# JuliaQuantumControl/GRAPE.jl

Hardware: AMD Instinct MI355X
Metric: GRAPE gradient evals/sec (N=64, 1000 steps, 128 traj) (higher is better)
Workload: dtype f64

## Files before the change

### grape.jl_amd/api.py

```python
from __future__ import annotations

import ctypes as C
import os
import subprocess
import sys

import numpy as np

_HERE = os.path.dirname(os.path.abspath(__file__))
_CSRC = os.path.join(_HERE, "csrc")
_LIBNAME = "libgrape_hip.so"

J_T_SM, J_T_SS, J_T_RE = 0, 1, 2
GRAD_GRADGEN, GRAD_TAYLOR = 0, 1
PROP_EXP, PROP_SERIES = 0, 1
ABI_VERSION = 7

STATUS = {0: "GRAPE_OK", -1: "GRAPE_ERR_INVALID", -2: "GRAPE_ERR_HIP", -3: "GRAPE_ERR_CHI_NORM",
          -4: "GRAPE_ERR_SINGULAR", -5: "GRAPE_ERR_TAYLOR", -6: "GRAPE_ERR_NO_CONTROLS", -7: "GRAPE_ERR_AGAIN",
          -8: "GRAPE_ERR_HOST"}

EXPORTS = ["grape_create", "grape_destroy", "grape_eval", "grape_forward", "grape_backward",
           "grape_forward_device", "grape_backward_device", "grape_check", "grape_get_propagator",
           "grape_get_tau_grads", "grape_get_storage", "grape_get_timings", "grape_reset_timings", "grape_get_work", "grape_get_cert_table", "grape_get_seg_table",
           "grape_last_error", "grape_abi_version", "grape_set_fused_sweeps", "grape_get_sums", "grape_backward_xi",
           "grape_get_final_states", "grape_backward_chi",
           "grape_get_time_gradient", "grape_set_tlist", "grape_eval_batch", "grape_get_batch_info", "grape_create_open",
           "grape_hvp", "grape_get_hvp_info", "grape_open_time_gradient", "grape_open_hvp", "grape_get_open_hvp_info",
           "grape_open_eval_batch", "grape_get_open_batch_info", "grape_open_set_running_cost", "grape_open_backward_xi",
           "grape_hvp_forward", "grape_hvp_backward", "grape_hvp_backward_chi",
           "grape_open_hvp_forward", "grape_open_hvp_backward", "grape_open_hvp_backward_chi",
           "grape_expect", "grape_get_expect_info"]


class GrapeHipError(RuntimeError):
    def __init__(self, code, msg):
        super().__init__(f"{STATUS.get(code, code)}: {msg}")
        self.code = code


class _Problem(C.Structure):
    _fields_ = [("abi_version", C.c_int32), ("N", C.c_int32), ("L", C.c_int32), ("K", C.c_int32),
                ("K_total", C.c_int32), ("N_T", C.c_int32), ("functional", C.c_int32),
                ("gradient_method", C.c_int32), ("hc_per_traj", C.c_int32), ("device", C.c_int32),
                ("tlist", C.c_void_p), ("H0", C.c_void_p), ("Hc", C.c_void_p), ("shape", C.c_void_p),
                ("psi0", C.c_void_p), ("target", C.c_void_p), ("weights", C.c_void_p),
                ("chi_min_norm", C.c_double), ("taylor_max_order", C.c_int32),
                ("taylor_tolerance", C.c_double),
                ("Dpen", C.c_void_p), ("dpen_per_traj", C.c_int32), ("lambda_b", C.c_double),
                ("prop_method", C.c_int32), ("prop_tolerance", C.c_double),
                ("ndev", C.c_int32), ("devices", C.c_void_p), ("taylor_no_check", C.c_int32)]


class _Lindblad(C.Structure):
    _fields_ = [("J", C.c_int32), ("cops_per_traj", C.c_int32), ("cops", C.c_void_p)]


def library_path() -> str:
    return os.path.join(_CSRC, _LIBNAME)


def build_asm(verbose: bool = False, workdir: str | None = None) -> str:
    asm_dir = os.path.join(_CSRC, "asm")
    work = workdir or asm_dir
    kernels = (("gen_t16.py", "expm_t16_asm"), ("gen_t16q.py", "expm_t16q_asm"), ("gen_t16p.py", "expm_t16p_asm"), ("gen_t16p.py", "expm_t16p4_asm"), ("gen_t18g.py", "expm_t18g_asm"), ("gen_t18gp.py", "expm_t18gp_asm"), ("gen_d3.py", "deriv3_asm"), ("gen_d3s.py", "deriv3s_asm"), ("gen_d3s.py", "deriv3g_asm"),
               ("gen_lg.py", "lg_gemm_asm"), ("gen_d4.py", "deriv4_asm_128"), ("gen_d4.py", "deriv4_asm_256"))
    co_path, emb_s, emb_o = os.path.join(work, "grape_asm.co"), os.path.join(work, "asm_embed.S"), os.path.join(work, "asm_embed.o")
    llvm = "/opt/rocm/lib/llvm/bin"
    cmds, objs = [], []
    for gen_py, name in kernels:
        s_path, o_path = os.path.join(work, name + ".s"), os.path.join(work, name + ".o")
        gen = subprocess.run([sys.executable, os.path.join(asm_dir, gen_py), s_path], capture_output=True, text=True)
        if verbose or gen.returncode:
            print(gen.stdout, gen.stderr)
        if gen.returncode:
            raise RuntimeError(gen_py + " failed")
        cmds.append([os.path.join(llvm, "clang"), "-x", "assembler", "-target", "amdgcn-amd-amdhsa", "-mcpu=gfx950", "-c", s_path, "-o", o_path])
        objs.append(o_path)
    cmds.append([os.path.join(llvm, "ld.lld"), "-shared"] + objs + ["-o", co_path])
    with open(emb_s, "w") as f:
        f.write('\t.section .rodata\n\t.globl grape_asm_co_start\n\t.globl grape_asm_co_end\n\t.p2align 12\n'
                'grape_asm_co_start:\n\t.incbin "grape_asm.co"\ngrape_asm_co_end:\n\t.byte 0\n'
                '\t.section .note.GNU-stack,"",@progbits\n')
    cmds.append(["gcc", "-c", "-fPIC", "asm_embed.S", "-o", "asm_embed.o"])
    for c in cmds:
        res = subprocess.run(c, capture_output=True, text=True, cwd=work)
        if verbose or res.returncode:
            print(" ".join(c), res.stdout, res.stderr)
        if res.returncode:
            raise RuntimeError("assembling the gfx950 kernels failed")
    return emb_o


def _sources():
    srcs = [os.path.join(_CSRC, f) for f in ("grape_hip.hip", "grape_t18.hip", "grape_kernels.hip.h", "grape_large.hip.h",
                                             "grape_series.hip.h", "grape_cheby.hip.h", "grape_t18.hip.h", "grape_t18_coeffs.h",
                                             "grape_deriv3.hip.h", "grape_timegrad.hip.h", "grape_batch.hip.h", "grape_lindblad.hip.h", "grape_lindblad_tg.hip.h", "grape_hvp.hip.h", "grape_hvp_split.hip.h", "grape_lindblad_hvp.hip.h", "grape_lindblad_hvp_split.hip.h", "grape_lindblad_batch.hip.h", "grape_lindblad_rc.hip.h", "grape_devmem.h", "grape_cert.hip.h", "grape_expect.hip.h", "grape_econ_coeffs.h", os.path.join("asm", "gen_t16.py"), os.path.join("asm", "gen_t16q.py"), os.path.join("asm", "gen_t16p.py"), os.path.join("asm", "gen_t18g.py"), os.path.join("asm", "gen_t18gp.py"), os.path.join("asm", "gen_d3.py"), os.path.join("asm", "gen_d3s.py"), os.path.join("asm", "gen_lg.py"), os.path.join("asm", "gen_d4.py"), os.path.join("asm", "gcn.py"))]
    return srcs, os.path.join(_HERE, "..", "include", "grape_hip.h")


def _up_to_date(out: str) -> bool:
    srcs, hdr = _sources()
    return os.path.exists(out) and all(os.path.getmtime(out) >= os.path.getmtime(s) for s in srcs + [hdr])


def build_library(force: bool = False, verbose: bool = False, extra_flags=(), out: str | None = None) -> str:
    import fcntl
    import shutil
    import tempfile
    out = out or library_path()
    if not force and _up_to_date(out):
        return out
    srcs, _ = _sources()
    with open(os.path.join(_CSRC, ".build.lock"), "w") as lockf:
        fcntl.flock(lockf, fcntl.LOCK_EX)
        if not force and _up_to_date(out):
            return out
        work = tempfile.mkdtemp(prefix="_build_", dir=_CSRC)
        procs = []
        try:
            base = ["hipcc", "--offload-arch=gfx950", "-O3", "-std=c++17", "-fPIC", "-Wno-unused-value"] + list(extra_flags)
            objs = [os.path.join(work, "grape_hip.o"), os.path.join(work, "grape_t18.o")]
            cmds = [base + ["-cuid=grapehip0", "-c", srcs[0], "-o", objs[0]],
                    base + ["-cuid=grapehip1", "-mllvm", "-amdgpu-mfma-vgpr-form", "-c", srcs[1], "-o", objs[1]]]
            procs = [subprocess.Popen(c, stdout=subprocess.PIPE, stderr=subprocess.STDOUT, text=True) for c in cmds]
            objs.append(build_asm(verbose, workdir=work))
            outs = [p.communicate()[0] for p in procs]
            if verbose or any(p.returncode for p in procs):
                print("\n".join(outs))
            if any(p.returncode for p in procs):
                raise RuntimeError("hipcc failed building " + out)
            tmp_so = os.path.join(work, _LIBNAME)
            res = subprocess.run(["hipcc", "--offload-arch=gfx950", "-shared", "-fPIC"] + objs + ["-o", tmp_so], capture_output=True, text=True)
            if verbose or res.returncode:
                print(res.stdout, res.stderr)
            if res.returncode:
                raise RuntimeError("hipcc failed linking " + out)
            asm_dir = os.path.join(_CSRC, "asm")
            for f in os.listdir(work):
                if f.endswith(".s") or f.endswith(".co"):
                    os.replace(os.path.join(work, f), os.path.join(asm_dir, f))
            os.replace(tmp_so, out)
        finally:
            for p in procs:
                if p.poll() is None:
                    p.kill()
                    p.communicate()
            shutil.rmtree(work, ignore_errors=True)
    return out


_lib = None


def load_library():
    global _lib
    if _lib is not None:
        return _lib
    path = library_path()
    if not os.path.exists(path):
        raise GrapeHipError(-2, f"{path} not built; run __graft_entry__.build() (no CPU fallback exists)")
    try:
        import torch
    except ImportError:
        pass
    lib = C.CDLL(path)
    vp, dp, ip = C.c_void_p, C.POINTER(C.c_double), C.c_int
    lib.grape_create.argtypes = [C.POINTER(vp), C.POINTER(_Problem)]
    lib.grape_create_open.argtypes = [C.POINTER(vp), C.POINTER(_Problem), C.POINTER(_Lindblad)]
    lib.grape_destroy.argtypes = [vp]
    lib.grape_destroy.restype = None
    lib.grape_eval.argtypes = [vp, vp, dp, vp, vp, vp]
    lib.grape_forward.argtypes = [vp, vp, vp]
    lib.grape_backward.argtypes = [vp, vp, vp]
    lib.grape_forward_device.argtypes = [vp, vp, vp, vp]
    lib.grape_backward_device.argtypes = [vp, vp, vp, vp]
    lib.grape_check.argtypes = [vp, vp]
    lib.grape_get_propagator.argtypes = [vp, ip, ip, vp]
    lib.grape_get_tau_grads.argtypes = [vp, vp]
    lib.grape_get_storage.argtypes = [vp, ip, vp]
# ... 251 lines not shown

    def hvp_forward(self, V, final_states=False):
        v, nv = self._hvp_dirs(V)
        dtau = np.empty((nv, self.K), dtype=np.complex128)
        dsums = np.empty(nv, dtype=np.complex128)
        dpsi = np.empty((nv, self.K, self.N), dtype=np.complex128) if final_states else None
        self._chk(self._lib.grape_hvp_forward(self._h, nv, v.ctypes.data, dtau.ctypes.data, dsums.ctypes.data,
                                              dpsi.ctypes.data if final_states else None))
        if v.ndim == 1:
            dtau, dsums, dpsi = dtau[0], dsums[0], (dpsi[0] if final_states else None)
        return (dtau, dsums, dpsi) if final_states else (dtau, dsums)

    def hvp_backward(self, f_total, df_total):
        one = np.ndim(df_total) == 0
        df = np.ascontiguousarray(df_total, dtype=np.complex128)
        if np.ndim(df_total) > 1 or df.size == 0:
            raise ValueError(f"df_total must be a complex scalar or [nv] with nv >= 1, got {np.shape(df_total)}")
        nv = df.size
        out = np.empty((nv, self.L * self.N_T))
        f = np.array([complex(f_total).real, complex(f_total).imag], dtype=np.float64)
        self._chk(self._lib.grape_hvp_backward(self._h, nv, f.ctypes.data, df.ctypes.data, out.ctypes.data))
        return out[0] if one else out

    def hvp_backward_chi(self, chi, dchi):
        chi = np.ascontiguousarray(chi, dtype=np.complex128)
        d = np.ascontiguousarray(dchi, dtype=np.complex128)
        if chi.shape != (self.K, self.N):
            raise ValueError(f"chi must be [K, N] = [{self.K}, {self.N}], got {chi.shape}")
        if d.ndim not in (2, 3) or d.shape[-2:] != (self.K, self.N) or d.size == 0:
            raise ValueError(f"dchi must be [K, N] = [{self.K}, {self.N}] or [nv, {self.K}, {self.N}] with nv >= 1, got {d.shape}")
        nv = 1 if d.ndim == 2 else d.shape[0]
        out = np.empty((nv, self.L * self.N_T))
        self._chk(self._lib.grape_hvp_backward_chi(self._h, nv, chi.ctypes.data, d.ctypes.data, out.ctypes.data))
        return out[0] if d.ndim == 2 else out

    def set_tlist(self, tlist):
        t = np.ascontiguousarray(tlist, dtype=np.float64)
        if t.shape != (self.N_T + 1,):
            raise ValueError(f"tlist must have N_T + 1 = {self.N_T + 1} points, got {t.shape}")
        self._chk(self._lib.grape_set_tlist(self._h, t.ctypes.data))
        self._tlist = t

    def forward_device(self, d_pulsevals_ptr, d_out_ptr, stream=0):
        self._chk(self._lib.grape_forward_device(self._h, d_pulsevals_ptr, d_out_ptr, stream))

    def backward_device(self, d_f_ptr, d_G_ptr, stream=0):
        self._chk(self._lib.grape_backward_device(self._h, d_f_ptr, d_G_ptr, stream))

    def set_fused_sweeps(self, on=True):
        return bool(self._lib.grape_set_fused_sweeps(self._h, int(bool(on))))

    def check(self, stream=0):
        self._chk(self._lib.grape_check(self._h, stream))

    def propagator(self, k, n):
        out = np.empty((self.N, self.N), dtype=np.complex128)
        self._chk(self._lib.grape_get_propagator(self._h, k, n, out.ctypes.data))
        return out.T.copy()

    def tau_grads(self):
        out = np.empty((self.K, self.L, self.N_T), dtype=np.complex128)
        self._chk(self._lib.grape_get_tau_grads(self._h, out.ctypes.data))
        return out

    def storage(self, which=0):
        out = np.empty((self.K, self.N_T + 1, self.N), dtype=np.complex128)
        self._chk(self._lib.grape_get_storage(self._h, which, out.ctypes.data))
        return out

    def timings(self):
        ms = np.full(8, -1.0)
        self._lib.grape_get_timings(self._h, ms.ctypes.data, 8)
        out = dict(zip(["expm", "forward", "backward", "deriv", "reduce", "total"], ms[:6].tolist()))
        if ms[6] >= 0.0:
            out["host_enqueue"] = float(ms[6])
        if ms[7] >= 0.0:
            out["gradient_allreduce_us"] = float(ms[7]) * 1e3
        return out

    def reset_timings(self):
        self._chk(self._lib.grape_reset_timings(self._h))

    def work(self):
        w = np.zeros(22)
        self._lib.grape_get_work(self._h, w.ctypes.data, 22)
        return dict(cells=w[0], squarings=w[1], flop_expm=w[2], flop_deriv=w[3], deriv_orders=w[4],
                    pivoted_cells=w[5], expm_cells=w[6], series_terms=w[7], series_steps=w[8],
                    t18_mfma_flop=w[9], t18_squarings=w[10], t18_cells=w[11], matrix_free_fallback=w[12], t16_cells=w[13],
                    asm_kernel=w[14], asm_deriv_kernel=w[15], asm_blocked_products=w[16],
                    walk_steps=w[17], scan_block=w[18], t16_certified=w[19], seg_certified=w[20], t16q_cells=w[21])

    def cert_table(self):
        dims = np.zeros(3, np.int32)
        self._chk(self._lib.grape_get_cert_table(self._h, dims.ctypes.data, None, None))
        KC, n8, n6 = (int(x) for x in dims)
        coef, exps = np.zeros((KC, n8 + n6)), np.zeros(n8 + n6, np.int32)
        if n8 + n6:
            self._chk(self._lib.grape_get_cert_table(self._h, dims.ctypes.data, coef.ctypes.data, exps.ctypes.data))
        ex = np.stack([(exps >> (4 * l)) & 15 for l in range(self.L)], axis=1) if n8 + n6 else np.zeros((0, self.L), np.int32)
        return coef[:, :n8], coef[:, n8:], ex

    def seg_table(self):
        dims = np.zeros(4, np.int32)
        self._chk(self._lib.grape_get_seg_table(self._h, dims.ctypes.data, None, None))
        KC, n4, n8, n12 = (int(x) for x in dims)
        nt = n4 + n8 + n12
        coef, exps = np.zeros((KC, nt)), np.zeros(nt, np.int32)
        if nt:
            self._chk(self._lib.grape_get_seg_table(self._h, dims.ctypes.data, coef.ctypes.data, exps.ctypes.data))
        ex = np.stack([(exps >> (4 * l)) & 15 for l in range(self.L)], axis=1) if nt else np.zeros((0, self.L), np.int32)
        return coef[:, :n4], coef[:, n4:n4 + n8], coef[:, n4 + n8:], ex


def liouvillian(H, cops=()):
    H = np.asarray(H, dtype=np.complex128)
    d = H.shape[0]
    if H.shape != (d, d):
        raise ValueError(f"H must be [d, d], got {H.shape}")
    eye = np.eye(d)
    heff = H.copy()
    for A in cops:
        A = np.asarray(A, dtype=np.complex128)
        heff = heff - 0.5j * (A.conj().T @ A)
    out = np.kron(eye, heff) - np.kron(heff.conj(), eye)
    for A in cops:
        A = np.asarray(A, dtype=np.complex128)
        out = out + 1j * np.kron(A.conj(), A)
    return out


class GrapeHipOpen(GrapeHip):

    def __init__(self, H0, Hc, cops, tlist, rho0, target, weights=None, functional=J_T_SM, shape=None, K_total=None,
                 device=0, chi_min_norm=0.0, prop_tolerance=0.0):
        self._lib = load_library()
        H0 = np.asarray(H0)
        if H0.ndim != 3 or H0.shape[1] != H0.shape[2]:
            raise ValueError(f"H0 must be [K, d, d], got {H0.shape}")
        K, N = H0.shape[0], H0.shape[1]
        Hc = np.asarray(Hc)
        per_traj = Hc.ndim == 4
        if Hc.ndim not in (3, 4) or Hc.shape[-2:] != (N, N) or (per_traj and Hc.shape[0] != K):
            raise ValueError(f"Hc must be [L, d, d] or [K, L, d, d] with d = {N}, K = {K}, got {Hc.shape}")
        L = Hc.shape[1] if per_traj else Hc.shape[0]
        tlist = np.ascontiguousarray(tlist, dtype=np.float64)
        if tlist.ndim != 1 or len(tlist) < 2:
            raise ValueError("tlist must hold at least two time points")
        N_T = len(tlist) - 1
        if weights is not None and np.shape(weights) != (K,):
            raise ValueError(f"weights must be [K] = [{K}], got {np.shape(weights)}")
        cops = None if cops is None or np.size(cops) == 0 else np.asarray(cops)
        cops_per_traj = cops is not None and cops.ndim == 4
        if cops is not None and (cops.ndim not in (3, 4) or cops.shape[-2:] != (N, N) or (cops_per_traj and cops.shape[0] != K)):
            raise ValueError(f"cops must be [J, d, d] or [K, J, d, d] with d = {N}, K = {K}, got {cops.shape}")
        self.N, self.L, self.K, self.N_T = N, L, K, N_T
        self.J = 0 if cops is None else cops.shape[-3]
        self.K_total = K if K_total is None else int(K_total)
        self.functional = functional
        self.prop_method = PROP_EXP
        self.lambda_b = 0.0
        self._H0 = _c128(np.swapaxes(H0, -1, -2), (K, N, N))
        self._Hc = _c128(np.swapaxes(Hc, -1, -2))
        self._cops = None if cops is None else _c128(np.swapaxes(cops, -1, -2))
        self._psi0 = _c128(np.swapaxes(np.asarray(rho0), -1, -2), (K, N, N))
        self._target = None if target is None else _c128(np.swapaxes(np.asarray(target), -1, -2), (K, N, N))
        self._tlist = tlist
        self._weights = None if weights is None else np.ascontiguousarray(weights, dtype=np.float64)
        self._shape = None if shape is None else np.ascontiguousarray(shape, dtype=np.float64).reshape(L, N_T)
        p = _Problem()
        p.abi_version = ABI_VERSION
        p.N, p.L, p.K, p.K_total, p.N_T = N, L, K, self.K_total, N_T
        p.functional, p.gradient_method, p.hc_per_traj, p.device = functional, GRAD_GRADGEN, int(per_traj), device
        p.tlist = self._tlist.ctypes.data
# ... 164 lines not shown
```

### grape.jl_amd/csrc/asm/gen_t16.py

```python
import os
import re
import struct
import sys
from types import SimpleNamespace

sys.path.insert(0, os.path.dirname(os.path.abspath(__file__)))
from gcn import Prog, Reg, V, A, S, VCC, EXEC, Neg, Abs, kernel_text
from gcn import HZ_MFMA_TO_VALU as gcn_wait_valu, HZ_MFMA_TO_MEM as gcn_wait_mem

NT = 4
NP = 64
LDB = (3 * NP + 2) * 8
PLB = NP * 8
TROW = 16 * LDB
PLANES = NP * LDB
E1 = PLANES
EXH = 256 * 8 + 128
EXW = 2 * EXH
E2 = E1 + 4 * EXW
RED = E2 + 4 * EXW
XS0 = RED + 16 * 8
XS1 = XS0 + 1024
LDS_BYTES = XS1 + 1024
KERNARG = 136
# ... 230 lines not shown
        p.valu("v_mul_u32_u24", self.v_CM, LDB, vpc)
        p.valu("v_and_b32", vpc, 1, vy)
        p.valu("v_lshlrev_b32", vpc, 3, vpc)
        p.valu("v_lshrrev_b32", vx, 1, vy)
        p.valu("v_add_u32", vpc, vpc, vx)
        p.valu("v_lshl_add_u32", self.v_CM, vpc, 3, self.v_CM)
        for r in range(4):
            p.valu("v_add_u32", vx, 4 * r, vrg)
            p.v_cmp("v_cmp_eq_u32", self.s_dmask[r], vx, vc)
        self.load_constants()
        p.s_waitcnt(lgkm=0)
        wg = S(2)
        t0, t1, t2 = self.s_tmp[0], self.s_tmp[1], self.s_tmp[2]
        p.salu("s_mul_i32", t2, self.s_KC, self.s_NT)
        p.s_load(2, self.s_t0, self.s_karg, 72)
        p.s_load(1, self.s_tmp[3], self.s_t0, 24)
        p.salu("s_lshl_b32", self.s_tmp[3], self.s_tmp[3], 2)
        p.s_cmp("s_cmp_gt_u32", self.s_tmp[3], t2)
        p.s_branch("s_cbranch_scc1", "L_end")
        if self.diag:
            p.s_load(2, self.s_diag, self.s_karg, 64)
            p.salu("s_lshl_b32", t0, wg, 2)
            p.salu("s_add_u32", t0, t0, self.s_wave)
            p.salu("s_mul_i32", t0, t0, 8 * self.NSTAMP)
            p.s_waitcnt(lgkm=0)
            p.salu("s_add_u32", self.s_diag.sub(0), self.s_diag.sub(0), t0)
            p.salu("s_addc_u32", self.s_diag.sub(1), self.s_diag.sub(1), 0)
        p.s_load(2, self.s_t1, self.s_karg, 80)
        p.salu("s_lshl_b32", t0, wg, 4)
        ent = S(60, 4)
        p.s_load(4, ent, self.s_t1, t0)
        p.s_load(1, t1, self.s_karg, 60)
        p.s_waitcnt(lgkm=0)
        p.salu("s_mov_b32", self.s_cell, ent.sub(0))
        p.salu("s_mov_b32", self.s_end, ent.sub(1))
        p.salu("s_mov_b32", self.s_step, ent.sub(2))
        p.salu("s_mov_b32", self.s_idx, 0)
        p.s_cmp("s_cmp_eq_u32", self.s_end, 0)
        p.s_branch("s_cbranch_scc1", "L_end")
        p.salu("s_and_b32", t1, t1, 1)
        p.s_cmp("s_cmp_eq_u32", self.s_step, 1)
        p.salu("s_cselect_b32", t1, t1, 0)
        p.salu("s_lshl_b32", self.s_tflip, t1, 31)
        p.salu("s_mov_b32", self.s_prop, 0)
        p.salu("s_mov_b32", self.s_prog, 0)
        p.salu("s_mov_b32", self.s_xs, XS0)
        p.salu("s_mov_b32", self.s_pm, 0)
        if not self.diag:
            p.s_load(2, self.s_splan, self.s_karg, 128)
        p.s_load(1, self.s_scell, self.s_karg, 124)
        q, r, i = self.s_kc, self.s_n, t0
        p.salu("s_mov_b32", q, 0)
        p.salu("s_mov_b32", r, 0)
        p.salu("s_mov_b32", i, 31)
        p.label("L_div")
        p.salu("s_lshl_b32", r, r, 1)
        p.salu("s_lshr_b32", t1, self.s_cell, i)
        p.salu("s_and_b32", t1, t1, 1)
        p.salu("s_or_b32", r, r, t1)
        p.s_cmp("s_cmp_ge_u32", r, self.s_NT)
        p.s_branch("s_cbranch_scc0", "L_div_skip")
        p.salu("s_sub_u32", r, r, self.s_NT)
        p.salu("s_lshl_b32", t1, 1, i)
        p.salu("s_or_b32", q, q, t1)
        p.label("L_div_skip")
        p.salu("s_sub_u32", i, i, 1)
        p.s_cmp("s_cmp_ge_i32", i, 0)
        p.s_branch("s_cbranch_scc1", "L_div")
        p.valu("v_lshlrev_b32", vx, 10, vrg)
        p.valu("v_lshl_add_u32", vx, vc, 4, vx)
        p.salu("s_lshl_b32", self.s_tmp[0], self.s_wave, 8)
        p.valu("v_add_u32", vx, self.s_tmp[0], vx)
        p.valu("v_lshl_add_u32", vy, vw, 4, vc)
        p.valu("v_lshlrev_b32", vy, 10, vy)
        p.valu("v_lshl_add_u32", vy, vrg, 4, vy)
        p.s_cmp("s_cmp_lg_u32", self.s_tflip, 0)
        p.salu("s_cselect_b64", VCC, -1, 0)
        for r_ in range(4):
            p.valu("v_add_u32", vidx, 4096 * r_, vx)
            p.valu("v_add_u32", vpc, 64 * r_, vy)
            p.valu("v_cndmask_b32", self.v_UO[r_], vidx, vpc, VCC)
        self.vp.free(t)

    early_free = False

    def pf_alloc(self):
        return [self.ap.alloc(2) for _ in range(5)]

    def pf_late(self, pf):
        pass

    def fetch_plan(self, pf, ki):
        if 0 <= ki < 10:
            self.fetch(ki // 2, pf[ki // 2], half=ki % 2)

    def load_constants(self):
        for i in range(1, 16):
            self.smov64(self.s_c[i], self.c[f"C{i}"])

    def cell_bases_issue(self, kc, n, cell):
        p = self.p
        t0, t1 = self.s_tmp[0], self.s_tmp[1]
        if self.diag:
            p.salu("s_mov_b32", self.s_snext, 0)
        else:
            p.salu("s_lshl_b32", t0, cell, 2)
            p.s_load(1, self.s_snext, self.s_splan, t0)
        p.s_cmp("s_cmp_lg_u64", self.s_rep, 0)
        p.salu("s_cselect_b32", self.s_t0.sub(0), self.s_rep.sub(0), self.s_dts.sub(0))
        p.salu("s_cselect_b32", self.s_t0.sub(1), self.s_rep.sub(1), self.s_dts.sub(1))
        p.salu("s_lshl_b32", t0, kc, 2)
        p.salu("s_cselect_b32", t0, t0, 0)
        p.s_load(1, self.s_k, self.s_t0, t0)
        p.salu("s_lshl_b32", t0, n, 3)
        p.s_load(2, self.s_dt, self.s_dts, t0)
        self.s_base(n, cell)

    def s_base(self, n, cell):
        p = self.p
        t0, t1 = self.s_tmp[0], self.s_tmp[1]
        p.s_cmp("s_cmp_lg_u32", self.s_scell, 0)
        p.salu("s_cselect_b32", t1, cell, n)
        p.salu("s_lshl_b32", t0, t1, 16)
        p.salu("s_lshr_b32", t1, t1, 16)
        p.salu("s_add_u32", self.s_sb.sub(0), self.s_Sf.sub(0), t0)
        p.salu("s_addc_u32", self.s_sb.sub(1), self.s_Sf.sub(1), t1)

    def cell_bases_finish(self, kc):
        p = self.p
        t0, t1 = self.s_tmp[0], self.s_tmp[1]
        p.s_waitcnt(lgkm=0)
        p.s_cmp("s_cmp_lg_u64", self.s_rep, 0)
        p.salu("s_cselect_b32", self.s_k, self.s_k, kc)
        p.salu("s_lshl_b32", t0, self.s_k, 16)
        p.salu("s_lshr_b32", t1, self.s_k, 16)
        p.salu("s_add_u32", self.s_hb.sub(0), self.s_H0.sub(0), t0)
        p.salu("s_addc_u32", self.s_hb.sub(1), self.s_H0.sub(1), t1)
        p.salu("s_and_b32", t0, self.s_snext, SQ_MASK)
        p.salu("s_lshl_b32", t0, t0, 20)
        p.salu("s_sub_u32", self.s_dt.sub(1), self.s_dt.sub(1), t0)

    def cell_bases(self, kc, n, cell):
        self.cell_bases_issue(kc, n, cell)
        self.cell_bases_finish(kc)

    def fetch(self, u, dst, half=None):
        p = self.p
        (i0, j0), (i1, j1) = TILES[2 * u], TILES[2 * u + 1]
        toff = self.s_tmp[2]
        p.s_cmp("s_cmp_lt_u32", self.s_wave, 2)
        self.ssel(toff, (16 * i0 * NP + 16 * j0) * 8, (16 * i1 * NP + 16 * j1) * 8)
        if half in (None, 0):
            p.salu("s_add_u32", self.s_t0.sub(0), self.s_hb.sub(0), toff)
            p.salu("s_addc_u32", self.s_t0.sub(1), self.s_hb.sub(1), 0)
            p.global_load(4, dst.sub(0, 4), self.v_GO, self.s_t0)
            p.global_load(4, dst.sub(4, 4), self.v_GOI, self.s_t0)
        if half in (None, 1):
            p.salu("s_add_u32", self.s_t1.sub(0), self.s_sb.sub(0), toff)
            p.salu("s_addc_u32", self.s_t1.sub(1), self.s_sb.sub(1), 0)
            p.global_load(4, dst.sub(8, 4), self.v_GO, self.s_t1)
            p.global_load(4, dst.sub(12, 4), self.v_GOI, self.s_t1)

    def commit(self, pf, fill=None):
        self.p.tag = "commit"
        self._commit(pf, fill)
        self.p.tag = ""

    def _commit(self, pf, fill=None):
        p = self.p
        ta, tb, tc = self.vp.alloc(), self.vp.alloc(), self.vp.alloc()
        dtT = S(self.s_tmp[4].idx, 2)
        p.salu("s_mov_b32", dtT.sub(0), self.s_dt.sub(0))
        p.salu("s_xor_b32", dtT.sub(1), self.s_dt.sub(1), self.s_tflip)
        for u in range(5):
            src = pf[u]
            hr, hi_, sr, si = ta.sub(0, 4), ta.sub(4, 4), tb.sub(0, 4), tb.sub(4, 4)
            for j, dst in enumerate((hr, hi_, sr, si)):
                for e in range(4):
                    p.valu("v_accvgpr_read_b32" if src.cls == "a" else "v_mov_b32", dst.sub(e), src.sub(4 * j + e))
            ar, ai, sm = tc.sub(0, 4), hr, hi_
            xr0, xr1, xi0, xi1 = sr.d(0), sr.d(1), si.d(0), si.d(1)
            p.valu("v_add_f64", xr0, hr.d(0), sr.d(0))
            p.valu("v_add_f64", xr1, hr.d(1), sr.d(1))
            p.valu("v_add_f64", xi0, hi_.d(0), si.d(0))
            p.valu("v_add_f64", xi1, hi_.d(1), si.d(1))
            p.valu("v_mul_f64", ar.d(0), dtT, xi0)
            p.valu("v_mul_f64", ar.d(1), dtT, xi1)
            p.valu("v_mul_f64", ai.d(0), Neg(self.s_dt), xr0)
            p.valu("v_mul_f64", ai.d(1), Neg(self.s_dt), xr1)
            p.valu("v_add_f64", sm.d(0), ar.d(0), ai.d(0))
            p.valu("v_add_f64", sm.d(1), ar.d(1), ai.d(1))
            (i0, j0), (i1, j1) = TILES[2 * u], TILES[2 * u + 1]
            va, vm = tc.sub(4), tc.sub(5)
            p.s_cmp("s_cmp_lt_u32", self.s_wave, 2)
            self.ssel(self.s_tmp[0], 16 * j0 * LDB + 16 * i0 * 8, 16 * j1 * LDB + 16 * i1 * 8)
            self.ssel(self.s_tmp[1], 16 * i0 * LDB + 16 * j0 * 8, 16 * i1 * LDB + 16 * j1 * 8)
            p.valu("v_add_u32", va, self.s_tmp[0], self.v_CP)
            p.valu("v_add_u32", vm, self.s_tmp[1], self.v_CM)
            cstep = (8 if self.PCOL_PERM else 1) * LDB
            for e in range(2):
                p.ds_write(64, va, ar.d(e), e * cstep)
                p.ds_write(64, va, ai.d(e), e * cstep + PLB)
                p.ds_write(64, va, sm.d(e), e * cstep + 2 * PLB)
            d0, d1 = i0 == j0, i1 == j1
            if not (d0 and d1):
                nar, ms = sr, si
                p.valu("v_mul_f64", nar.d(0), ar.d(0), -1.0)
                p.valu("v_mul_f64", nar.d(1), ar.d(1), -1.0)
                p.valu("v_add_f64", ms.d(0), ai.d(0), Neg(ar.d(0)))
                p.valu("v_add_f64", ms.d(1), ai.d(1), Neg(ar.d(1)))
                if d0 or d1:
                    p.salu("s_mov_b64", self.s_save, EXEC)
                    p.s_cmp("s_cmp_lt_u32", self.s_wave, 2)
                    lab = f"L_mirror_{u}_{len(p.ins)}"
                    p.s_branch("s_cbranch_scc1" if d0 else "s_cbranch_scc0", lab)
                for e in range(2):
                    p.ds_write(64, vm, nar.d(e), 32 * e)
                    p.ds_write(64, vm, ai.d(e), 32 * e + PLB)
                    p.ds_write(64, vm, ms.d(e), 32 * e + 2 * PLB)
                if d0 or d1:
                    p.label(lab)
            if fill:
                fill(u)
        for t in (ta, tb, tc):
            self.vp.free(t)

    def product(self, Q, B, half_last=False, init=None, hook=None, bload=None, fused=None):
        p = self.p
        NS = len(Q)
        started = set(init or ())

        def nslots(sk):
            return NS - 1 if (half_last and 2 * sk >= NT) else NS

        def rd(pl, so, sk, r):
            p.tag = "fragment"
            p.ds_read(64, self.aop[pl][so], self.v_AA[so][sk], self.KSTEP * r * LDB + pl * PLB)
            p.tag = ""

        def mma(so, pl, a, b):
            acc = Q[so][pl]
            c = acc if (so, pl) in started else 0
            started.add((so, pl))
            p.mfma(acc, a, b, c)

        sk0 = 0
        if fused:
            assert not bload and (NS == 4 or (NS == 3 and half_last))

            def rdk(pl, so, r):
                p.tag = "fragment"
                p.ds_read(64, self.aop[pl][r], self.v_AA[so][0], self.KSTEP * r * LDB + pl * PLB)
                p.tag = ""

            fused["valu"](0)
            for st in fused["stores"](0):
                st()
            if fused.get("after_first"):
                fused["after_first"]()
            for r in range(4):
                for pl in range(3):
                    rdk(pl, 0, r)
            for so in range(NS):
                gaps = [[] for _ in range(12)]
                if so < 3:
                    fused["valu"](so + 1)
                    pend = list(fused["stores"](so + 1))
                    for q, st in enumerate(pend):
                        gaps[4 * (q // 2) + (q % 2)].append(st)
                    last = {pl: (4 * pl + 1 if pend else 0) for pl in range(3)}
                    for r in range(4 if so + 1 < NS else 0):
                        for pl in range(3):
                            gaps[max(last[pl], 3 * r + pl)].append(lambda pl=pl, r=r: rdk(pl, so + 1, r))
                j = 0
                for r in range(4):
                    for pl in range(3):
                        mma(so, pl, self.aop[pl][r], B[pl][0].d(r))
                        for f in gaps[j]:
                            f()
                        j += 1
            if fused.get("post"):
                fused["post"]()
            p.s_barrier()
            sk0 = 1
        for pl in range(3):
            for so in range(nslots(sk0)):
                rd(pl, so, sk0, 0)
            if bload:
                bload(pl, sk0, 0)
        for sk in range(sk0, 4):
            for r in range(4):
                ns = nslots(sk)
                more = not (sk == 3 and r == 3)
                nsk, nr = (sk, r + 1) if r < 3 else (sk + 1, 0)
                nsn = nslots(nsk) if more else 0
                for pl in range(3):
                    for so in range(ns):
                        mma(so, pl, self.aop[pl][so], B[pl][sk].d(r))
                        if hook and pl == 0 and so == 0:
                            hook(sk, r)
                    for so in range(nsn):
                        rd(pl, so, nsk, nr)
                    if bload and more:
                        bload(pl, nsk, nr)

    def plane_stores(self, sl, xr, xi, xs):
        if self.opts.get("nostore"):
            return []
        a = self.v_SA[sl]

        def st(h, pl, x):
            self.p.tag = "strip store"
            self.p.ds_write(128, a, x.sub(4 * h, 4), 16 * h + pl * PLB)
            self.p.tag = ""
        return [lambda h=h, pl=pl, x=x: st(h, pl, x) for pl, x in enumerate((xr, xi, xs)) for h in range(2)]

    def interleave(self, streams):
        streams = [list(s) for s in streams]
        if self.opts.get("serial"):
            for s in streams:
                for f in s:
                    f()
            return
        while any(streams):
            for s in streams:
                if s:
                    s.pop(0)()

    def acc_read(self, dst, src):
        if self.opts.get("noacc"):
            self.p.valu("v_mov_b32", dst.sub(0), dst.sub(0))
            self.p.valu("v_mov_b32", dst.sub(1), dst.sub(1))
            return
        self.p.valu("v_accvgpr_read_b32", dst.sub(0), src.sub(0))
        self.p.valu("v_accvgpr_read_b32", dst.sub(1), src.sub(1))

    def acc_write(self, dst, src):
        if self.opts.get("noacc"):
            self.p.valu("v_mov_b32", src.sub(0), src.sub(0))
            self.p.valu("v_mov_b32", src.sub(1), src.sub(1))
            return
        self.p.valu("v_accvgpr_write_b32", dst.sub(0), src.sub(0))
        self.p.valu("v_accvgpr_write_b32", dst.sub(1), src.sub(1))

    def wave_reduce(self, x, tmp, op):
        p = self.p
        for ctrl, rm in (("quad_perm:[1,0,3,2]", 0xF), ("quad_perm:[2,3,0,1]", 0xF), ("row_half_mirror", 0xF), ("row_mirror", 0xF),
                         ("row_bcast:15", 0xA), ("row_bcast:31", 0xC)):
            if rm != 0xF:
                p.valu("v_mov_b32", tmp.sub(0), 0)
                p.valu("v_mov_b32", tmp.sub(1), 0 if op == "v_add_f64" else 0xFFF00000)
            p.dpp_mov(tmp.sub(0), x.sub(0), ctrl, row_mask=rm)
            p.dpp_mov(tmp.sub(1), x.sub(1), ctrl, row_mask=rm)
            p.valu(op, x, x, tmp)

    def second_product_fork(self, cx):
        pass

    def second_product_square(self, cx, L_join):
        pass

    def cell_coeffs(self, q):
        return None

    def load_c16(self, k16):
        self.smov64(k16, self.c["C16"])

    def cell(self):
        p, c = self.p, self.s_c
        vp, ap = self.vp, self.ap
        Qt = [[V(8 * self.QT[3 * so + j], 8) for j in range(3)] for so in range(4)]
        for t in self.QT:
            vp.free_tiles.remove(t)
        Uprev = V(8 * self.UT, 64)
        for t in range(self.UT, self.UT + 8):
            vp.free_tiles.remove(t)

        self.stamp(0)
        self.As_re, self.As_im, self.As_sm = ap.alloc(4), ap.alloc(4), ap.alloc(4)
        As = (self.As_re, self.As_im, self.As_sm)

        def hook_store(sk, r):
            p.salu("s_mov_b64", self.s_save, EXEC)
            p.s_cmp("s_cmp_lg_u32", self.s_pm, 0)
            p.salu("s_cselect_b64", EXEC, -1, 0)
            p.global_store(4, self.v_UO[r], Uprev.sub(16 * sk + 4 * r, 4), self.s_ub[sk], nt=self.nt_u)
            p.salu("s_mov_b64", EXEC, self.s_save)

        def bload_A(pl, sk, r):
            if r % 2 == 0:
                p.tag = "strip load"
                p.ds_read(128, As[pl].sub(8 * sk + 2 * r, 4), self.v_SA[sk], 8 * r + pl * PLB)
                p.tag = ""

        B_As = [[S_.sub(8 * sl, 8) for sl in range(4)] for S_ in As]
        self.product(Qt[:3], B_As, half_last=True, hook=hook_store, bload=bload_A)
        ap.free(self.As_sm)
        vp.free(Uprev)
        self.stamp(1)
        As_re, As_im = self.As_re, self.As_im

        def A_(sl, r):
            return As_re.sub(8 * sl, 8).d(r), As_im.sub(8 * sl, 8).d(r)

        def in_place_y(sl_list):
            streams = []
            for sl in sl_list:
                for r in range(4):
                    p1, p2, p3 = (Qt[sl][j].d(r) for j in range(3))
                    streams.append([lambda p3=p3, p1=p1: p.valu("v_add_f64", p3, p3, Neg(p1)),
                                    lambda p1=p1, p2=p2: p.valu("v_add_f64", p1, p1, Neg(p2)),
                                    lambda p3=p3, p2=p2: p.valu("v_add_f64", p3, p3, Neg(p2))])
            for g in range(0, len(streams), 4):
                self.interleave(streams[g:g + 4])

        A2re, A2im, A2sm = [vp.alloc() for _ in range(4)], [vp.alloc() for _ in range(4)], [vp.alloc() for _ in range(4)]
        streams = []
        for sl in range(3):
            for r in range(4):
                p1, p2, p3 = (Qt[sl][j].d(r) for j in range(3))
                re_, im_ = A2re[sl].d(r), A2im[sl].d(r)
                streams.append([lambda re_=re_, p1=p1, p2=p2: p.valu("v_add_f64", re_, p1, Neg(p2)),
                                lambda im_=im_, p3=p3, p1=p1: p.valu("v_add_f64", im_, p3, Neg(p1)),
                                lambda im_=im_, p2=p2: p.valu("v_add_f64", im_, im_, Neg(p2))])
        for g in range(0, len(streams), 4):
            self.interleave(streams[g:g + 4])
        for r in range(4):
            p.ds_write(64, self.v_EW2, A2re[2].d(r), 128 * r)
            p.ds_write(64, self.v_EW2, A2im[2].d(r), EXH + 128 * r)
            p.ds_write(64, self.v_EW1, A2re[1].d(r), 128 * r)
            p.ds_write(64, self.v_EW1, A2im[1].d(r), EXH + 128 * r)
        p.s_waitcnt(lgkm=0)
        p.s_barrier()
        cx = SimpleNamespace(Qt=Qt, A2re=A2re, A2im=A2im, A2sm=A2sm)
        self.second_product_fork(cx)
        self.advance()
        self.cell_bases_issue(self.s_nkc, self.s_nn, self.s_ncell)
        txr, txi = vp.alloc(), vp.alloc()
        for h in range(2):
            p.ds_read(128, txr.sub(4 * h, 4), self.v_ER, 16 * h)
            p.ds_read(128, txi.sub(4 * h, 4), self.v_ER, EXH + 16 * h)
            p.ds_read(128, A2re[3].sub(4 * h, 4), self.v_ER, (E2 - E1) + 16 * h)
            p.ds_read(128, A2im[3].sub(4 * h, 4), self.v_ER, (E2 - E1) + EXH + 16 * h)
        self.stamp(2)
        tt = [vp.alloc(), vp.alloc()]

        def valu2(sl):
            if sl == 2:
                for r in range(4):
                    p.valu("v_add_f64", A2re[2].d(r), A2re[2].d(r), txr.d(r))
                    p.valu("v_add_f64", A2im[2].d(r), A2im[2].d(r), Neg(txi.d(r)))
                for r in range(4):
                    p.valu("v_mul_f64", A2im[3].d(r), A2im[3].d(r), -1.0)
                vp.free(txr)
                vp.free(txi)
            streams = []
            for r in range(4):
                xr, xi, xs = tt[0].d(r), tt[1].d(r), Qt[sl][1].d(r)
                a2r, a2i = A2re[sl].d(r), A2im[sl].d(r)
                ar_, ai_ = A_(sl, r)
                streams.append([lambda xr=xr, ar_=ar_: self.acc_read(xr, ar_),
                                lambda xi=xi, ai_=ai_: self.acc_read(xi, ai_),
                                lambda xr=xr: p.valu("v_mul_f64", xr, c[2], xr),
                                lambda xi=xi: p.valu("v_mul_f64", xi, c[2], xi),
                                lambda xr=xr, a2r=a2r: p.valu("v_fma_f64", xr, c[1], a2r, xr),
                                lambda xi=xi, a2i=a2i: p.valu("v_fma_f64", xi, c[1], a2i, xi),
                                lambda xs=xs, xr=xr, xi=xi: p.valu("v_add_f64", xs, xr, xi),
                                lambda r=r, a2r=a2r, a2i=a2i: p.valu("v_add_f64", A2sm[sl].d(r), a2r, a2i)])
            self.interleave(streams)

        self.product(Qt, [A2re, A2im, A2sm], fused={"valu": valu2, "stores": lambda sl: self.plane_stores(sl, tt[0], tt[1], Qt[sl][1]),
                                                    "post": self.cell_coeffs(False)})
        for t in tt + A2sm:
            vp.free(t)
        self.cell_bases_finish(self.s_nkc)
        self.stamp(3)
        uid = len(p.ins)
        L_cert, L_cert2, L_ones, L_vdone = f"L_cert_{uid}", f"L_cert2_{uid}", f"L_ones_{uid}", f"L_vdone_{uid}"
        p.salu("s_and_b32", self.s_tmp[0], self.s_scur, CERT_BIT)
        p.s_branch("s_cbranch_scc1", L_cert)
        facc, gacc, cacc = vp.alloc(), vp.alloc(), vp.alloc()
        for acc in (facc, gacc, cacc):
            for j in range(8):
                p.valu("v_mov_b32", acc.sub(j), 0)
        streams = []
        for sl in range(4):
            for r in range(4):
                k = len(streams) % 4
                p1, p2, p3 = (Qt[sl][j].d(r) for j in range(3))
                a2r, a2i = A2re[sl].d(r), A2im[sl].d(r)
                f, g_, cs = facc.d(k), gacc.d(k), cacc.d(k)
                streams.append([
                    lambda p3=p3, p1=p1: p.valu("v_add_f64", p3, p3, Neg(p1)),
                    lambda p1=p1, p2=p2: p.valu("v_add_f64", p1, p1, Neg(p2)),
                    lambda p3=p3, p2=p2: p.valu("v_add_f64", p3, p3, Neg(p2)),
                    lambda cs=cs, a2r=a2r: p.valu("v_add_f64", cs, cs, Abs(a2r)),
                    lambda f=f, p1=p1: p.valu("v_fma_f64", f, p1, p1, f),
                    lambda g_=g_, a2r=a2r, p1=p1: p.valu("v_fma_f64", g_, a2r, p1, g_),
                    lambda cs=cs, a2i=a2i: p.valu("v_add_f64", cs, cs, Abs(a2i)),
                    lambda f=f, p3=p3: p.valu("v_fma_f64", f, p3, p3, f),
                    lambda g_=g_, a2i=a2i, p3=p3: p.valu("v_fma_f64", g_, a2i, p3, g_)])
        for g in range(0, 16, 4):
            self.interleave(streams[g:g + 4])
        f, g_, cs = facc.d(0), gacc.d(0), cacc.d(0)
        for k in range(1, 4):
            p.valu("v_add_f64", f, f, facc.d(k))
            p.valu("v_add_f64", g_, g_, gacc.d(k))
            p.valu("v_add_f64", cs, cs, cacc.d(k))
        ones, ct = cacc.d(1), vp.alloc(1)
        lo, hi = dbits(1.0)
        p.valu("v_mov_b32", ones.sub(0), lo)
        p.valu("v_mov_b32", ones.sub(1), hi)
        p.label(L_ones)
        p.mfma(ct, ones, cs, 0)
        p.salu("s_and_b32", self.s_tmp[0], self.s_scur, CERT_BIT)
        p.s_branch("s_cbranch_scc1", L_cert2)
# ... 559 lines not shown
```

### grape.jl_amd/csrc/asm/gen_t16q.py

```python
import os
import re
import sys

sys.path.insert(0, os.path.dirname(os.path.abspath(__file__)))
from gcn import S, Neg, kernel_text
import gen_t16 as g16
from gen_t16 import E1, E2, EXH, LDS_BYTES, KERNARG

HERE = os.path.dirname(os.path.abspath(__file__))
Q_BIT = 0x200
MFMA_Q = 120 + 120 + 2 * 192 + 1


def t16q_coeffs():
    txt = open(os.path.join(HERE, "..", "grape_t18_coeffs.h")).read()
    c = {}
    for m in re.finditer(r"#define\s+T16Q_(C\d+|THETA)\s+([-+0-9.eE]+)", txt):
        c[m.group(1)] = float(m.group(2))
    assert len(c) == 17 and c["C2"] == 0.0, c
    return c


class GenQ(g16.Gen):
    def __init__(self, name="expm_t16q_asm", **kw):
        super().__init__(name=name, **kw)
        self.cq = t16q_coeffs()

    def cell_coeffs(self, q):
        c = self.cq if q else self.c

        def load():
            for i in range(3, 16):
                self.smov64(self.s_c[i], c[f"C{i}"])
        return load

    def load_c16(self, k16):
        p = self.p
        lo, hi = g16.dbits(self.c["C16"])
        qlo, qhi = g16.dbits(self.cq["C16"])
        p.salu("s_and_b32", self.s_tmp[4], self.s_scur, Q_BIT)
        self.ssel(k16.sub(0), qlo, lo)
        self.ssel(k16.sub(1), qhi, hi)

    def second_product_fork(self, cx):
        p = self.p
        uid = len(p.ins)
        cx.L_q = f"L_q_{uid}"
        cx.pool = list(self.vp.free_tiles)
        p.salu("s_and_b32", self.s_tmp[0], self.s_scur, Q_BIT)
        p.s_branch("s_cbranch_scc1", cx.L_q)

    def second_product_square(self, cx, L_join):
        p, vp = self.p, self.vp
        Qt, A2re, A2im, A2sm = cx.Qt, cx.A2re, cx.A2im, cx.A2sm
        p.s_branch("s_branch", L_join)
        p.label(cx.L_q)
        joined = list(vp.free_tiles)
        vp.free_tiles[:] = cx.pool

        self.advance()
        self.cell_bases_issue(self.s_nkc, self.s_nn, self.s_ncell)
        txr, txi = vp.alloc(), vp.alloc()
        for h in range(2):
            p.ds_read(128, txr.sub(4 * h, 4), self.v_ER, 16 * h)
            p.ds_read(128, txi.sub(4 * h, 4), self.v_ER, EXH + 16 * h)
            p.ds_read(128, A2re[3].sub(4 * h, 4), self.v_ER, (E2 - E1) + 16 * h)
            p.ds_read(128, A2im[3].sub(4 * h, 4), self.v_ER, (E2 - E1) + EXH + 16 * h)
        self.stamp(2)
        tx1 = (txr, txi)

        def valu(sl):
            if sl == 2:
                for r in range(4):
                    p.valu("v_add_f64", A2re[2].d(r), A2re[2].d(r), tx1[0].d(r))
                    p.valu("v_add_f64", A2im[2].d(r), A2im[2].d(r), Neg(tx1[1].d(r)))
                for r in range(4):
                    p.valu("v_mul_f64", A2im[3].d(r), A2im[3].d(r), -1.0)
                vp.free(tx1[0])
                vp.free(tx1[1])
            for r in range(4):
                p.valu("v_add_f64", A2sm[sl].d(r), A2re[sl].d(r), A2im[sl].d(r))

        self.product(Qt[:3], [A2re, A2im, A2sm], half_last=True,
                     fused={"valu": valu, "stores": lambda sl: self.plane_stores(sl, A2re[sl], A2im[sl], A2sm[sl]),
                            "post": self.cell_coeffs(True)})
        for t in A2sm:
            vp.free(t)
        self.cell_bases_finish(self.s_nkc)
        self.stamp(3)
        kq = S(58, 2)
        self.smov64(kq, self.cq["C1"])
        streams = []
        for sl in range(3):
            for r in range(4):
                p1, p2, p3 = (Qt[sl][j].d(r) for j in range(3))
                streams.append([lambda p3=p3, p1=p1: p.valu("v_add_f64", p3, p3, Neg(p1)),
                                lambda p1=p1, p2=p2: p.valu("v_add_f64", p1, p1, Neg(p2)),
                                lambda p3=p3, p2=p2: p.valu("v_add_f64", p3, p3, Neg(p2)),
                                lambda p1=p1: p.valu("v_mul_f64", p1, kq, p1),
                                lambda p3=p3: p.valu("v_mul_f64", p3, kq, p3)])
        for g in range(0, len(streams), 4):
            self.interleave(streams[g:g + 4])
        for r in range(4):
            p.ds_write(64, self.v_EW2, Qt[2][0].d(r), 128 * r)
            p.ds_write(64, self.v_EW2, Qt[2][2].d(r), EXH + 128 * r)
            p.ds_write(64, self.v_EW1, Qt[1][0].d(r), 128 * r)
            p.ds_write(64, self.v_EW1, Qt[1][2].d(r), EXH + 128 * r)
        p.s_waitcnt(lgkm=0)
        p.s_barrier()
        txr, txi = vp.alloc(), vp.alloc()
        for h in range(2):
            p.ds_read(128, txr.sub(4 * h, 4), self.v_ER, 16 * h)
            p.ds_read(128, txi.sub(4 * h, 4), self.v_ER, EXH + 16 * h)
            p.ds_read(128, Qt[3][0].sub(4 * h, 4), self.v_ER, (E2 - E1) + 16 * h)
            p.ds_read(128, Qt[3][2].sub(4 * h, 4), self.v_ER, (E2 - E1) + EXH + 16 * h)
        drop = vp.alloc()
        p.mfma(drop, A2re[0].d(0), A2re[0].d(0), 0)
        vp.free(drop)
        for r in range(4):
            p.valu("v_add_f64", Qt[2][0].d(r), Qt[2][0].d(r), txr.d(r))
            p.valu("v_add_f64", Qt[2][2].d(r), Qt[2][2].d(r), Neg(txi.d(r)))
        for r in range(4):
            p.valu("v_mul_f64", Qt[3][2].d(r), Qt[3][2].d(r), -1.0)
        vp.free(txr)
        vp.free(txi)
        p.salu("s_and_b32", self.s_prop, self.s_prop, 1)
        self.stamp(4)
        assert sorted(vp.free_tiles) == sorted(joined), (vp.free_tiles, joined)


def generate(path=None, **kw):
    g = GenQ(**kw)
    prog = g.build()
    text = kernel_text(prog, KERNARG, LDS_BYTES)
    if path:
        with open(path, "w") as f:
            f.write(text)
    return g, prog, text


if __name__ == "__main__":
    out = sys.argv[1] if len(sys.argv) > 1 else os.path.join(HERE, "expm_t16q_asm.s")
    g, prog, _ = generate(out)
    print(f"{out}: {len(prog.ins)} lines, {prog.count('mfma')} matrix instructions, {prog.count('valu') + prog.count('dpp')} vector, "
          f"{prog.count('lds')} LDS, {prog.count('vmem')} global, {prog.auto_nops} wait states inserted")
```

### grape.jl_amd/csrc/grape_hip.hip

```cpp
#include "../../include/grape_hip.h"
#include "grape_kernels.hip.h"
#include "grape_t18_coeffs.h"
#include "grape_econ_coeffs.h"
#include "grape_large.hip.h"
#include "grape_series.hip.h"
#include "grape_cheby.hip.h"
#include "grape_timegrad.hip.h"
#include "grape_lindblad.hip.h"
#include "grape_lindblad_tg.hip.h"
#include "grape_hvp.hip.h"
#include "grape_hvp_split.hip.h"
#include "grape_lindblad_hvp.hip.h"
#include "grape_lindblad_hvp_split.hip.h"
#include "grape_lindblad_batch.hip.h"
#include "grape_lindblad_rc.hip.h"
#include "grape_devmem.h"
#include "grape_cert.hip.h"
#include "grape_expect.hip.h"

#include <rccl/rccl.h>
#include <dlfcn.h>
#include <mutex>

#include <algorithm>
// ... 16 lines not shown
    try {
        *err = std::string("host-side C++ exception caught at the C boundary: ") + what;
    } catch (...) {
    }
    return -8;
}
#define GRAPE_BARRIER(errptr)                                                                                   \
    catch (const std::bad_alloc &) { return barrier_fail((errptr), "std::bad_alloc (out of host memory)"); }    \
    catch (const std::exception &e) { return barrier_fail((errptr), e.what()); }                                \
    catch (...) { return barrier_fail((errptr), "unknown exception"); }

void test_throw_point(const char *where) {
    const char *hk = getenv("GRAPE_TEST_HOOKS");
    if (!(hk && atoi(hk) == 1)) return;
    const char *t = getenv("GRAPE_TEST_THROW"), *at = getenv("GRAPE_TEST_THROW_AT");
    if (!t || strcmp(at ? at : "early", where)) return;
    if (!strcmp(t, "bad_alloc")) throw std::bad_alloc();
    throw std::runtime_error(t);
}

constexpr int kRing = 64;
constexpr int kPhases = 6;
struct Phase { hipEvent_t e0, e1; bool used; };

}

struct OpenCtx;

struct grape_handle {
    grape_problem p{};
    int N = 0, NP = 0, NT = 0, L = 0, K = 0, K_total = 0, N_T = 0;
    int device = 0;
    hipStream_t stream = nullptr;
    double *d_H0f = nullptr, *d_Hcf = nullptr, *d_H0t = nullptr, *d_Hct = nullptr;
    double *d_H0p = nullptr, *d_Hcp = nullptr, *d_vecs = nullptr;
    double *d_H0q = nullptr, *d_Hcq = nullptr, *d_park2 = nullptr;
    double *d_H0q3 = nullptr, *d_Hcq3 = nullptr, *d_H0p3 = nullptr, *d_Hcp3 = nullptr;
    int deriv4_blocks = 0;
    double *d_park3 = nullptr;
    int deriv3_blocks = 0, deriv3_wpt = 0;
    bool deriv3_h0g = false;
    bool deriv3_general = false;
    int deriv2 = 0, deriv2_maxm = 0;
    bool deriv_stream = false;
    bool deriv_stream_never = false;
    int deriv_blocks = 0;
    bool large = false;
    int chunk = 0;
    double *d_lg[9] = {nullptr, nullptr, nullptr, nullptr, nullptr, nullptr, nullptr, nullptr, nullptr};
    double *d_dinv = nullptr;
    int *d_scell = nullptr;
    double *d_colpart = nullptr;
    bool lg_form2 = false;
    double *d_normpart = nullptr;
    double *d_dts = nullptr, *d_shape = nullptr, *d_weights = nullptr;
    double2 *d_psi0 = nullptr, *d_target = nullptr;
    double *d_eps = nullptr;
    double2 *d_U = nullptr, *d_fw = nullptr, *d_bw = nullptr, *d_tg = nullptr;
    double *d_ret = nullptr;
    double *d_out = nullptr;
    double *d_f = nullptr, *d_G = nullptr, *d_rho = nullptr;
    int *d_flags = nullptr;
    int *d_cellflag = nullptr;
    int KC = 0;
    bool herm = false;
    bool herm_ctrl = false;
    bool t18 = false;
    bool t18_small = true;
    bool t16 = true;
    double *d_gram = nullptr;
    int *d_celllist = nullptr;
    double *d_cert = nullptr;
    int *d_cert_exp = nullptr;
    int cert_n8 = 0, cert_n6 = 0;
    double *d_seg = nullptr;
    double *d_seg8 = nullptr;
    int *d_seg_exp = nullptr;
    int seg_n8 = 0, seg_n4 = 0, seg_n12 = 0, seg8_stride = 0, seg_exp_off = 0;
    int *d_segplan = nullptr;
    double *d_t86 = nullptr, *d_t412 = nullptr;
    int *d_texp = nullptr;
    int t_n8 = 0, t_n6 = 0, t_n4 = 0, t_n12 = 0;
    bool asm16q = false;
    bool t16q_twin = false;
    bool asm16 = false;
    bool asm16p = false;
    double *d_dte = nullptr;
    bool asm18gp = false;
    bool asm18g = false;
    int *d_wgtab = nullptr, *d_prog = nullptr, *d_splan = nullptr;
    double2 *d_xinit = nullptr;
    int asm_blocks = 0;
    int last_walk_fuse = 0;
    bool asm_sq = true;
    int asm_walk = 0;
    bool foreign_stream = false;
    bool credit_pending = false;
    std::vector<double> bal;
    std::vector<double> bal_stage_chi, bal_stage_xi;
    double *d_Sf = nullptr;
    bool expm_persist = true;
    int expm_lds_pad_kb = 0;
    bool test_hooks = false;
    bool lg_asm = true;
    bool deriv3_asm = true;
    bool taylor_check = true;
    bool no_target = false;
    std::vector<int> cls;
    int *d_cls = nullptr, *d_rep = nullptr;
    int coop_S = 0;
    int *d_xcc_sw = nullptr;
    int coop_rpw = 0, coop_nw = 0;
    double2 *d_Dt = nullptr, *d_xi = nullptr;
    double *d_wq = nullptr, *d_gb = nullptr;
    bool have_gb = false;
    const double2 *xi_user = nullptr;
    double lambda_user = 0.0;
    unsigned long long *d_stats = nullptr;
    double *h_pin = nullptr;
    double *h_get = nullptr;
    DeviceBufs mem;
    size_t h_pin_doubles = 0;
    Phase ph[kRing][kPhases]{};
    long n_fwd = 0, n_bwd = 0;
    std::string err;
    bool have_forward = false, in_eval = false;
    double chi_min_norm = 1e-100, taylor_tol = 1e-16;
    int taylor_max_order = 100;
    bool fuse = false;
    bool fuse_on = true;
    bool want_bw = true;
    bool bw_done = false;
    bool bw_unit = false;
    bool z_valid = false;
    double *d_inv_tnorm = nullptr, *d_ones = nullptr;
    double2 *d_z = nullptr;
    bool scan16 = false;
    int scan_Bk = 0, scan_NB = 0;
    double2 *d_scanF = nullptr, *d_scan_fw = nullptr, *d_scan_bw = nullptr;
    int num_cus = 256;
    bool series = false;
    bool u_fallback = false;
    double *d_rb = nullptr;
    double series_tol = 1e-17, series_theta = 3.0;
    double *d_n1 = nullptr;
    double2 *d_gpark = nullptr;
    int *d_morder = nullptr;
    int maxp = 0;
    int *d_batchflag = nullptr;
    bool deriv_econ = false;
    const double *d_econ_pairs = nullptr;
    int *d_celldeg = nullptr;
    double sub_theta = 0.0;
    int sq_plan = 2;
    double2 *d_xch = nullptr;
    int *d_xcc = nullptr;
    int cheby_S = 0, cheby_round = 0, cheby_pair = 0;
    double2 *d_chi_in = nullptr;
    std::vector<grape_handle *> shards;
    std::vector<int> shard_lo;
    std::vector<int> shard_dev;
    bool use_rccl = false;
    void *comm_set = nullptr;
    std::vector<double *> d_red;
    bool rccl_fwd_checked = false, rccl_bwd_checked = false;
    hipEvent_t ar0 = nullptr, ar1 = nullptr;
// ... 2560 lines not shown
        size_t free_p = 0, total_p = 0;
        if (const char *envb = getenv("GRAPE_U_BUDGET_GB")) free_p = (size_t)(atof(envb) * 1073741824.0);
        else if (hipMemGetInfo(&free_p, &total_p) != hipSuccess) free_p = (size_t)-1;
        if (NP >= 48 && !h->large && h->deriv2 && h->series_tol <= h->taylor_tol && bytes <= ((size_t)24 << 30) &&
            (double)bytes <= 0.5 * (double)free_p && !(envp && atoi(envp) == 0)) {
            h->maxp = 32;
            CCHK(h->mem.alloc(&h->d_gpark, (size_t)K * N_T * h->maxp * NP));
            CCHK(h->mem.alloc(&h->d_morder, (size_t)K * N_T));
            CCHK(hipMemset(h->d_morder, 0xFF, (size_t)K * N_T * sizeof(int)));
        }
    }
    CCHK(h->mem.alloc(&h->d_fw, (size_t)K * (N_T + 1) * NP));
    CCHK(h->mem.alloc(&h->d_bw, (size_t)K * (N_T + 1) * NP));
    {
        const char *envs = getenv("GRAPE_SCAN16");
        if (const char *envs2 = getenv("GRAPE_SCAN")) envs = envs2;
        { const char *env1w = getenv("GRAPE_SWEEP1W"); g_sweep_wg32 = env1w && atoi(env1w) == 0; }
        const bool forced = envs && atoi(envs) != 0;
        const int kmax = NP == 16 ? 96 : NP == 32 ? 64 : NP == 48 ? 48 : 24;
        if (NP <= 64 && !h->series && !h->large && !(envs && atoi(envs) == 0) && N_T >= 8 && (forced || (h->KC <= kmax && N_T >= 64))) {
            const double t2 = NP == 16 ? 0.22 : NP == 32 ? 1.1 : 1.8, t1 = NP == 16 ? 0.45 : NP == 32 ? 3.3 : NP == 48 ? 7.3 : 13.5;
            const double slots = NP == 16 ? 16.0 * h->num_cus : (double)h->num_cus;
            int best = 4;
            double best_t = 1e300;
            for (int Bk = 4; Bk <= 64 && Bk < std::max(N_T, 5); Bk += (Bk < 16 ? 2 : 4)) {
                const int NBq = (N_T + Bk - 1) / Bk;
                const double t = std::ceil((double)h->KC * NBq / slots) * Bk * t1 + (NBq + Bk) * t2;
                if (t < best_t) { best_t = t; best = Bk; }
            }
            if (const char *envb = getenv("GRAPE_SCAN16_BK")) best = std::max(2, atoi(envb));
            h->scan_Bk = std::min(best, N_T);
            h->scan_NB = (N_T + h->scan_Bk - 1) / h->scan_Bk;
            CCHK(h->mem.alloc(&h->d_scanF, (size_t)h->KC * h->scan_NB * NP * NP));
            CCHK(h->mem.alloc(&h->d_scan_fw, (size_t)K * (h->scan_NB + 1) * NP));
            CCHK(h->mem.alloc(&h->d_scan_bw, (size_t)K * (h->scan_NB + 1) * NP));
            h->scan16 = true;
        }
    }
    CCHK(h->mem.alloc(&h->d_tg, (size_t)K * L * N_T));
    CCHK(h->mem.alloc(&h->d_ret, (size_t)2 * K + 8 + (size_t)L * N_T + 4 + (size_t)GRAPE_STAT_SHARDS * GRAPE_STAT_SLOTS));
    h->d_out = h->d_ret;
    h->d_G = h->d_ret + (size_t)2 * K + 8;
    h->d_flags = (int *)(h->d_G + (size_t)L * N_T);
    h->d_stats = (unsigned long long *)(h->d_G + (size_t)L * N_T + 4);
    CCHK(h->mem.alloc(&h->d_f, 2)); CCHK(h->mem.alloc(&h->d_rho, (size_t)K));
    CCHK(h->mem.alloc(&h->d_cellflag, (size_t)K * N_T));
    bool sf_per_cell_ok = false;
    const char *envp16 = getenv("GRAPE_EXPM_ASM16P");
    const bool p_direct = p->hc_per_traj && (h->herm ? L <= 4 : L <= 2) && !(envp16 && atoi(envp16) == 0);
    if (p->hc_per_traj && !p_direct && h->t18 && !h->large && !h->series && h->NT == 4) {
        size_t free_b = 0, total_b = 0;
        CCHK(hipMemGetInfo(&free_b, &total_b));
        const char *envs = getenv("GRAPE_SF_PER_CELL");
        sf_per_cell_ok = !(envs && atoi(envs) == 0) && 2.0 * (double)h->KC * N_T * NP * NP * 16.0 + 8e9 < (double)free_b;
    }
    const bool sf_shape_ok = !p->hc_per_traj || p_direct || sf_per_cell_ok;
    h->asm16 = h->asm16 && h->t16 && h->t18 && h->herm && !h->large && !h->series && h->NT == 4 && sf_shape_ok && (long)K * N_T < (1L << 28);
    h->asm18g = h->asm18g && h->t18 && !h->herm && !h->large && !h->series && h->NT == 4 && sf_shape_ok && (long)K * N_T < (1L << 28);
    h->asm16p = h->asm16 && p_direct;
    h->asm18gp = h->asm18g && p_direct;
    {
        const char *enve = getenv("GRAPE_DERIV_ECON");
        const bool lg_ok = h->large && h->t18 && h->herm && !h->series;
        const bool t16c_ok = h->t16 && h->t18 && h->herm && !h->large && !h->series && (h->NT >= 3 || (h->NT == 2 && h->t18_small));
        h->deriv_econ = (h->asm16 || lg_ok || t16c_ok) && p->gradient_method == GRAPE_GRAD_GRADGEN && h->taylor_tol >= 1e-16 && h->d_batchflag &&
                        !(enve && atoi(enve) == 0);
        if (h->deriv_econ) h->d_econ_pairs = grape_econ_pairs();
        if (h->deriv_econ && !h->d_econ_pairs) h->deriv_econ = false;
        if (h->deriv_econ && lg_ok) {
            CCHK(h->mem.alloc(&h->d_celldeg, (size_t)h->KC * N_T));
            CCHK(hipMemset(h->d_celldeg, 0, (size_t)h->KC * N_T * sizeof(int)));
        }
    }
    if (h->asm16p || h->asm18gp) CCHK(h->mem.alloc(&h->d_dte, (size_t)(L <= 2 ? 4 : 8) * N_T));
    if (h->t18 && !h->large && !h->series && ((L > 2 && !p->hc_per_traj) || (h->asm16 && !h->asm16p) || (h->asm18g && !h->asm18gp)) && (h->NT >= 3 || h->t18_small))
        CCHK(h->mem.alloc(&h->d_Sf, (size_t)(p->hc_per_traj ? (size_t)h->KC * N_T : (size_t)N_T) * 2 * NP * NP));
    if (h->asm16 || h->asm18g) {
        const long ncell = (long)h->KC * N_T;
        h->asm_blocks = (int)std::max<long>(1, std::min<long>(h->num_cus, ncell));
        {
            const char *envt = getenv("GRAPE_EXPM_T16Q");
            const bool eligible = h->asm16 && !h->asm16p && !p->hc_per_traj && L >= 1 && L <= 2;
            h->asm16q = eligible && (envt ? atoi(envt) != 0 : ncell >= (long)T16Q_MIN_WALK * h->asm_blocks);
        }
        std::vector<int> tab((size_t)4 * h->asm_blocks);
        grape_t16_walks(h->KC, N_T, h->asm_blocks, tab.data());
        CCHK(h->mem.alloc(&h->d_wgtab, tab.size()));
        CCHK(h->mem.alloc(&h->d_splan, (size_t)ncell));
        CCHK(hipMemset(h->d_splan, 0, (size_t)ncell * sizeof(int)));
        CCHK(hipMemcpy(h->d_wgtab, tab.data(), tab.size() * sizeof(int), hipMemcpyHostToDevice));
        const char *envw = getenv("GRAPE_EXPM_WALK"), *envq = getenv("GRAPE_EXPM_SQ");
        h->asm_sq = !(envq && atoi(envq) == 0);
        h->asm_walk = h->KC == K ? (envw ? atoi(envw) & 3 : 3) : 0;
        if (h->scan16) h->asm_walk = 0;
        if (h->asm_walk) {
            std::vector<double> xi((size_t)2 * K * 64 * 2, 0.0);
            for (int k = 0; k < K; ++k) {
                double n2 = 0.0;
                for (int i = 0; i < 2 * N; ++i) n2 += p->target[(size_t)k * 2 * N + i] * p->target[(size_t)k * 2 * N + i];
                const double itn = n2 > 0.0 ? 1.0 / std::sqrt(n2) : 0.0;
                for (int i = 0; i < N; ++i) {
                    xi[2 * ((size_t)k * 64 + i)] = p->psi0[2 * ((size_t)k * N + i)];
                    xi[2 * ((size_t)k * 64 + i) + 1] = p->psi0[2 * ((size_t)k * N + i) + 1];
                    xi[2 * ((size_t)(K + k) * 64 + i)] = p->target[2 * ((size_t)k * N + i)] * itn;
                    xi[2 * ((size_t)(K + k) * 64 + i) + 1] = -p->target[2 * ((size_t)k * N + i) + 1] * itn;
                }
            }
            CCHK(h->mem.alloc(&h->d_xinit, (size_t)2 * K * 64));
            CCHK(hipMemcpy(h->d_xinit, xi.data(), xi.size() * 8, hipMemcpyHostToDevice));
            CCHK(h->mem.alloc(&h->d_prog, (size_t)2 * K));
            CCHK(hipMemset(h->d_prog, 0, (size_t)2 * K * sizeof(int)));
        }
    }
    if (!h->asm16 && !h->asm18g && h->t16 && h->t18 && h->herm && !h->large && !h->series && h->NT == 4 && !p->hc_per_traj && L >= 1 && L <= 2 &&
        (long)K * N_T < (1L << 28)) {
        const char *envt = getenv("GRAPE_EXPM_T16Q");
        const long ncell = (long)h->KC * N_T, blocks = std::max<long>(1, std::min<long>(h->num_cus, ncell));
        h->t16q_twin = envt ? atoi(envt) != 0 : ncell >= (long)T16Q_MIN_WALK * blocks;
        if (h->t16q_twin) {
            CCHK(h->mem.alloc(&h->d_splan, (size_t)ncell));
            CCHK(hipMemset(h->d_splan, 0, (size_t)ncell * sizeof(int)));
        }
    }
    if (h->t16 && h->t18 && h->herm && !h->large && !h->series && (h->NT >= 3 || (h->NT == 2 && h->t18_small))) {
        CCHK(h->mem.alloc(&h->d_celllist, (size_t)K * N_T));
        const int M = L + 1, KCn = h->KC;
        const int GS = M * M + M;
        std::vector<double> gram((size_t)KCn * GS);
        std::vector<int> repk(KCn, -1);
        auto shape_factor = [&](const double *op, double fro2) {
            if (!(fro2 > 0.0)) return 1.0;
            std::vector<double> a2((size_t)2 * N * N), a4((size_t)2 * N * N);
            auto square = [&](const double *a, std::vector<double> &c) {
                std::fill(c.begin(), c.end(), 0.0);
                for (int j = 0; j < N; ++j)
                    for (int k = 0; k < N; ++k) {
                        const double br = a[2 * ((size_t)j * N + k)], bi = a[2 * ((size_t)j * N + k) + 1];
                        const double *ak = a + 2 * (size_t)k * N;
                        double *cj = &c[2 * (size_t)j * N];
                        for (int i = 0; i < N; ++i) {
                            cj[2 * i] += ak[2 * i] * br - ak[2 * i + 1] * bi;
                            cj[2 * i + 1] += ak[2 * i] * bi + ak[2 * i + 1] * br;
                        }
                    }
            };
            square(op, a2);
            square(a2.data(), a4);
            double m8 = 0.0;
            for (double x : a4) m8 += x * x;
            const double s8 = std::pow(m8, 0.125), semi = std::pow(3.5, 0.125) * 2.0 * std::sqrt(fro2 / (double)N);
            const double kap = s8 / semi;
            return std::isfinite(kap) && kap > 0.0 ? kap : 1.0;
        };
        std::vector<double> kap_shared((size_t)L, -1.0);
        for (int k = K - 1; k >= 0; --k) repk[h->cls.empty() ? k : h->cls[k]] = k;
        const size_t nn2 = (size_t)2 * N * N;
        for (int kc = 0; kc < KCn; ++kc) {
            const int k = repk[kc] < 0 ? kc : repk[kc];
            auto op = [&](int a) { return a == 0 ? p->H0 + (size_t)k * nn2 : p->Hc + ((size_t)(p->hc_per_traj ? k : 0) * L + (a - 1)) * nn2; };
            for (int a = 0; a < M; ++a)
                for (int b = a; b < M; ++b) {
                    const double *x = op(a), *y = op(b);
                    double sum = 0.;
                    for (size_t i = 0; i < nn2; ++i) sum += x[i] * y[i];
                    gram[(size_t)kc * GS + (size_t)a * M + b] = gram[(size_t)kc * GS + (size_t)b * M + a] = sum;
                }
// ... 167 lines not shown
    ea.ablate = getenv("GRAPE_DIAG_ABLATE") ? atoi(getenv("GRAPE_DIAG_ABLATE")) : 0;
    static unsigned long long *d_stamps = nullptr;
    if (getenv("GRAPE_DIAG_STAMPS")) {
        if (!d_stamps) hipMalloc((void **)&d_stamps, (size_t)h->K * h->N_T * 32 * 8);
        hipMemsetAsync(d_stamps, 0, (size_t)h->K * h->N_T * 32 * 8, s);
    }
    ea.stamps = d_stamps;
    hipMemcpyToSymbolAsync(HIP_SYMBOL(g_diag_slot_base), &d_stamps, sizeof(d_stamps), 0, hipMemcpyHostToDevice, s);
    grape_t18_set_stamps(d_stamps, (void *)s);
#endif
    hipError_t e = hipSuccess;
    int walk_fuse = 0;
    if (!h->series) {
        phase_begin(h, 0, s);
        if (h->large) {
            e = h->t18 ? expm_large_t18(h, s) : expm_large(h, s);
        } else {
            const long ncell = (long)ea.K * ea.N_T;
            const int per_cu = h->NT == 1 ? 10 : h->NT == 2 ? 4 : 1;
            const int t18_blocks = 8 * (int)std::max<long>(1, std::min<long>((long)(h->num_cus / 8) * per_cu, (ncell + 7) / 8));
            if (h->t18 && (h->NT >= 3 || h->t18_small)) {
                if (h->d_Sf) {
                    CtrlSumArgs ca{};
                    ca.Hcf = h->d_Hcf; ca.eps = h->d_eps; ca.shape = h->d_shape; ca.Sf = h->d_Sf;
                    ca.L = h->L; ca.N_T = h->N_T; ca.pp2 = 2 * h->NP * h->NP;
                    ca.per_traj = h->p.hc_per_traj ? 1 : 0; ca.rep = h->d_rep;
                    hipLaunchKernelGGL(ctrl_sum_kernel, dim3((unsigned)((ca.per_traj ? h->KC : 1) * h->N_T), std::max(1, ca.pp2 / 2 / 2048)), dim3(256), 0, s, ca);
                    HIPCHK(h, hipGetLastError());
                    ea.Sf = h->d_Sf;
                }
                const bool t16 = h->d_celllist != nullptr;
                ea.cell_list = h->d_celllist; ea.listed = 0;
                if (t16) {
                    T16PlanArgs pa{};
                    pa.gram = h->d_gram; pa.eps = h->d_eps; pa.shape = h->d_shape; pa.dts = h->d_dts; pa.flags = h->d_flags;
                    pa.KC = h->KC; pa.L = h->L; pa.N_T = h->N_T; pa.N = h->N;
                    pa.splan = ((h->asm16 && (h->asm_sq || h->d_cert || h->asm16q)) || h->t16q_twin) ? h->d_splan : nullptr;
                    pa.sq_on = (h->asm16 && h->asm_sq) ? 1 : 0;
                    pa.cert = h->d_t86; pa.cert_exp = h->d_t86 ? h->d_texp : nullptr; pa.n8 = h->t_n8; pa.n6 = h->t_n6;
                    pa.verdict = h->d_cellflag;
                    pa.seg = h->d_t412; pa.seg8 = h->d_seg8; pa.seg8_stride = h->seg8_stride; pa.seg8_exp = h->d_t412 ? h->d_texp : nullptr;
                    pa.seg_exp = h->d_t412 ? h->d_texp + h->t_n8 + h->t_n6 : nullptr;
                    pa.s8 = h->d_t412 ? h->t_n8 : 0; pa.n4 = h->t_n4; pa.n12 = h->t_n12; pa.segplan = h->d_segplan;
                    pa.cert_use = h->d_cert ? 1 : 0; pa.seg_use = h->d_seg ? 1 : 0; pa.q_use = (h->asm16q || h->t16q_twin) ? 1 : 0;
                    const unsigned plan_blocks = (unsigned)(h->KC * ((h->N_T + T16_PLAN_TPB - 1) / T16_PLAN_TPB));
                    const size_t plan_lds = t16_plan_lds(pa);
                    switch (plan_lds ? h->L : 0) {
                        case 1: hipLaunchKernelGGL(t16_plan_kernel<1>, dim3(plan_blocks), dim3(T16_PLAN_TPB), plan_lds, s, pa); break;
                        case 2: hipLaunchKernelGGL(t16_plan_kernel<2>, dim3(plan_blocks), dim3(T16_PLAN_TPB), plan_lds, s, pa); break;
                        case 3: hipLaunchKernelGGL(t16_plan_kernel<3>, dim3(plan_blocks), dim3(T16_PLAN_TPB), plan_lds, s, pa); break;
                        case 4: hipLaunchKernelGGL(t16_plan_kernel<4>, dim3(plan_blocks), dim3(T16_PLAN_TPB), plan_lds, s, pa); break;
                        default: hipLaunchKernelGGL(t16_plan_kernel<0>, dim3(plan_blocks), dim3(T16_PLAN_TPB), 0, s, pa); break;
                    }
                    HIPCHK(h, hipGetLastError());
                }
                const int blocks16 = (t16 && h->NT == 3) ? 8 * (int)std::max<long>(1, std::min<long>((long)(h->num_cus / 8) * 2, (ncell + 7) / 8)) : t18_blocks;
                h->credit_pending = false;
                if (h->asm18g) {
                    walk_fuse = h->asm_walk & (1 | ((h->fuse && h->fuse_on && h->want_bw) ? 2 : 0));
                    if (walk_fuse) HIPCHK(h, stream_fill(h->d_prog, 0, (size_t)2 * h->K * sizeof(int), s));
                    const void *walk[6] = {h->d_wgtab, h->d_xinit, h->d_fw, h->d_bw, h->d_prog, h->d_splan};
                    if (h->asm18gp) {
                        hipLaunchKernelGGL(dte_kernel, dim3((unsigned)((h->N_T + 255) / 256)), dim3(256), 0, s, (const double *)h->d_eps,
                                           (const double *)h->d_shape, (const double *)h->d_dts, h->L, h->N_T, 2, h->d_dte);
                        HIPCHK(h, hipGetLastError());
                    }
                    e = (hipError_t)grape_t18g_asm_launch(&ea, sizeof(ea), h->d_cellflag, (void *)s, h->asm_blocks, walk, walk_fuse, h->K,
                                                          h->asm18gp ? h->d_dte : nullptr);
                    h->credit_pending = !h->asm18gp;
                }
                else if (t16 && h->asm16p) {
                    walk_fuse = h->asm_walk & (1 | ((h->fuse && h->fuse_on && h->want_bw) ? 2 : 0));
                    if (walk_fuse) HIPCHK(h, stream_fill(h->d_prog, 0, (size_t)2 * h->K * sizeof(int), s));
                    hipLaunchKernelGGL(dte_kernel, dim3((unsigned)((h->N_T + 255) / 256)), dim3(256), 0, s, (const double *)h->d_eps,
                                       (const double *)h->d_shape, (const double *)h->d_dts, h->L, h->N_T, h->L <= 2 ? 2 : 4, h->d_dte);
                    HIPCHK(h, hipGetLastError());
                    const void *walk[6] = {h->d_wgtab, h->d_xinit, h->d_fw, h->d_bw, h->d_prog, h->d_splan};
                    e = (hipError_t)grape_t16p_asm_launch(&ea, sizeof(ea), h->d_cellflag, (void *)s, h->asm_blocks, walk, walk_fuse, h->K, h->d_dte);
                }
                else if (t16 && h->asm16) {
                    walk_fuse = h->asm_walk & (1 | ((h->fuse && h->fuse_on && h->want_bw) ? 2 : 0));
                    if (walk_fuse) HIPCHK(h, stream_fill(h->d_prog, 0, (size_t)2 * h->K * sizeof(int), s));
                    const void *walk[6] = {h->d_wgtab, h->d_xinit, h->d_fw, h->d_bw, h->d_prog, h->d_splan};
                    e = (hipError_t)grape_t16_asm_launch(&ea, sizeof(ea), h->d_cellflag, (void *)s, h->asm_blocks, walk, walk_fuse, h->K, h->asm16q ? 1 : 0);
                    h->credit_pending = true;
                }
                else {
                    ea.splan = h->t16q_twin ? h->d_splan : nullptr;
                    e = (hipError_t)grape_t18_launch(h->NT, h->herm ? 1 : 0, t16 ? 1 : 0, &ea, sizeof(ea), (void *)s, blocks16);
                }
                if (t16 && e == hipSuccess) {
                    ea.listed = 1;
                    e = (hipError_t)grape_t18_launch(h->NT, 1, 0, &ea, sizeof(ea), (void *)s, t18_blocks);
                }
            } else
            switch (h->NT) {
                case 1: e = launch_expm<1>(ea, h->herm, s, 0, h->expm_lds_pad_kb); break;
                case 2: e = launch_expm<2>(ea, h->herm, s, 0, h->expm_lds_pad_kb); break;
                case 3: e = launch_expm<3>(ea, h->herm, s, 0, h->expm_lds_pad_kb); break;
                default: {
                    const int nb = 8 * (h->num_cus / 8);
                    const bool persist = h->expm_persist && nb >= 8 && (long)ea.K * ea.N_T >= 4L * nb;
                    e = launch_expm<4>(ea, h->herm, s, persist ? nb : 0, h->expm_lds_pad_kb);
                    break;
                }
            }
        }
        HIPCHK(h, e);
        if (h->deriv_econ) {
            DerivEconArgs ec{};
            ec.verdict = h->d_cellflag; ec.splan = h->d_splan; ec.cls = h->d_cls; ec.flags = h->d_flags;
            ec.cell_deg = h->large ? h->d_celldeg : nullptr;
            ec.deg0 = ECON_DEG[ECON_VERDICT_SET]; ec.deg1 = ECON_DEG[ECON_NSETS - 1];
            ec.segplan = h->large ? nullptr : h->d_segplan; ec.deg_seg = ECON_DEG[0];
            static_assert(ECON_NSETS == 5, "segments 1.11 (three-moment certificate), 1.36 (verdict), 1.6, 2.0 (blocked path), 2.72 (one planned squaring)");
            ec.K = h->K; ec.KC = h->KC; ec.N_T = h->N_T; ec.batches_per_k = (h->N_T + 15) / 16;
            ec.nbatch_total = h->K * ec.batches_per_k; ec.batch_econ = h->d_batchflag + ec.nbatch_total;
            hipLaunchKernelGGL(deriv_econ_kernel, dim3((unsigned)((ec.nbatch_total + 255) / 256)), dim3(256), 0, s, ec);
            HIPCHK(h, hipGetLastError());
        }
        phase_end(h, 0, s);
    }
#ifdef GRAPE_DIAG
    if (ea.stamps) {
        hipStreamSynchronize(s);
        const size_t nb = (size_t)h->KC * h->N_T;
        std::vector<unsigned long long> st(nb * 32);
        hipMemcpy(st.data(), ea.stamps, nb * 32 * 8, hipMemcpyDeviceToHost);
        auto avg = [&](int i1, int i0) {
            double sum = 0;
            size_t cnt = 0;
            for (size_t b = 0; b < nb; ++b)
                if (st[b * 32 + i1] && st[b * 32 + i0]) { sum += (double)(st[b * 32 + i1] - st[b * 32 + i0]); ++cnt; }
            return cnt ? sum / cnt : 0.0;
        };
        if (h->t18 && h->NT >= 3) {
            const char *tn[] = {"form A (+norm)", "A2 = A A + half exchange", "A3 = A A2", "store A3, norm A2, barrier", "A6 = A3 A3",
                                "A6 exchanges + norms", "scaling, B1 -> X, barrier", "A9 = B1 B5", "+B4, B3+A9 -> X, B2", "p = B2 + (B3+A9) A9",
                                "squarings", "store U", "end barrier"};
            for (int j = 0; j < 13; ++j) fprintf(stderr, "  stamp %-28s %9.0f cycles\n", tn[j], avg(j + 1, j));
            fprintf(stderr, "  stamp %-28s %9.0f cycles\n", "TOTAL per cell", avg(13, 0));
        } else {
        const char *pn[] = {"form A", "norm", "A2", "A4,A6 (+store A2)", "store A6 + combos", "dual", "U=A*T"};
        for (int j = 0; j < 7; ++j) fprintf(stderr, "  stamp %-24s %9.0f cycles\n", pn[j], avg(11 + j, j ? 10 + j : 0));
        fprintf(stderr, "  stamp %-24s %9.0f cycles\n", "P,Q + first inversion", avg(5, 17));
        fprintf(stderr, "  stamp   barrier %6.0f, P/Q stores %6.0f, barrier %6.0f, strip loads + barrier + I_0 %6.0f\n", avg(26, 17), avg(27, 26), avg(28, 27), avg(5, 28));
        fprintf(stderr, "  stamp   strip loads + barrier %6.0f, then wave 0 (I_0) %6.0f, wave 1 (tiles + prefetch) %6.0f, wave 2 (prefetch) %6.0f\n", avg(22, 28), avg(29, 22), avg(30, 22), avg(31, 22));
        for (int j = 0; j < 4; ++j) fprintf(stderr, "  stamp solve step %d             %9.0f cycles\n", j, avg(6 + j, 5 + j));
        for (int j = 0; j < 1; ++j)
            fprintf(stderr, "  stamp   step %d, waves done after %6.0f %6.0f %6.0f %6.0f cycles\n", j, avg(18 + 4 * j, 5 + j),
                    avg(19 + 4 * j, 5 + j), avg(20 + 4 * j, 5 + j), avg(21 + 4 * j, 5 + j));
        fprintf(stderr, "  stamp %-24s %9.0f cycles\n", "squarings + store U", avg(4, 3));
        fprintf(stderr, "  stamp %-24s %9.0f cycles\n", "TOTAL per cell", avg(4, 0));
        }
    }
#endif
    h->last_walk_fuse = walk_fuse;
    h->tg_state = h->want_bw ? 2 : 1;
    h->ex_state = grape_handle::ExpectStore::READY;
    h->hvs.came(grape_handle::HvpSplit::EVAL);
    SweepArgs sa{};
    sa.U = h->d_U; sa.cls = h->d_cls; sa.psi0 = h->d_psi0; sa.target = h->d_target; sa.weights = h->d_weights;
    sa.store = h->d_fw; sa.tau = (double2 *)d_out; sa.f = nullptr; sa.rho = h->d_rho; sa.flags = h->d_flags;
    sa.chi_min_norm = h->chi_min_norm;
    sa.K = h->K; sa.K_total = h->K_total; sa.N = h->N; sa.N_T = h->N_T; sa.functional = h->p.functional;
    sa.xcc = h->d_xcc_sw;
    if (walk_fuse & 1) sa.resume = h->d_prog;
// ... 907 lines not shown
                               : "prop_method = GRAPE_PROP_SERIES is matrix-free: no propagator is materialised";
        return GRAPE_ERR_INVALID;
    }
    const size_t pp = (size_t)h->NP * h->NP;
    std::vector<double> tmp(2 * pp);
    const int rc = getter_fetch(h, tmp.data(), h->d_U + ((size_t)h->cls[k] * h->N_T + n) * pp, pp * 16);
    if (rc) return rc;
    for (int j = 0; j < h->N; ++j)
        for (int i = 0; i < h->N; ++i) {
            const double f = h->bal.empty() ? 1.0 : h->bal[i] / h->bal[j];
            out[2 * ((size_t)j * h->N + i)] = f * tmp[2 * ((size_t)i * h->NP + j)];
            out[2 * ((size_t)j * h->N + i) + 1] = f * tmp[2 * ((size_t)i * h->NP + j) + 1];
        }
    return GRAPE_OK;
}
GRAPE_BARRIER(h ? &h->err : &g_create_error)

int grape_get_timings(grape_handle *h, double *ms, int n) try {
    if (!h || !ms) return GRAPE_ERR_INVALID;
    if (h->open) {
        const OpenCtx *o = h->open;
        const double f = o->n_fwd ? o->ms_fwd / o->n_fwd : -1.0, b = o->n_bwd ? o->ms_bwd / o->n_bwd : -1.0;
        const double v[kPhases] = {0.0, f, b, 0.0, 0.0, f < 0.0 ? -1.0 : f + std::max(b, 0.0)};
        int cnt = 0;
        for (; cnt < kPhases && cnt < n; ++cnt) ms[cnt] = v[cnt];
        return cnt;
    }
    if (!h->shards.empty()) {
        int cnt = 0;
        for (size_t g = 0; g < h->shards.size(); ++g) {
            double cm[kPhases];
            cnt = grape_get_timings(h->shards[g], cm, n < kPhases ? n : kPhases);
            if (cnt < 0) return multi_fail(h, h->shards[g], cnt);
            for (int i = 0; i < cnt; ++i) ms[i] = g == 0 ? cm[i] : std::max(ms[i], cm[i]);
        }
        if (n > kPhases) { ms[kPhases] = h->host_enqueue_calls ? 2.0 * h->host_enqueue_ms / h->host_enqueue_calls : -1.0; cnt = kPhases + 1; }
        if (n > kPhases + 1) { ms[kPhases + 1] = (h->use_rccl && h->allreduce_calls) ? h->allreduce_ms / h->allreduce_calls : -1.0; cnt = kPhases + 2; }
        return cnt;
    }
    HIPCHK(h, hipSetDevice(h->device));
    HIPCHK(h, hipDeviceSynchronize());
    int cnt = 0;
    for (int i = 0; i < kPhases && i < n; ++i, ++cnt) {
        double sum = 0.0;
        int used = 0;
        for (int r = 0; r < kRing; ++r) {
            float t = 0.f;
            Phase &p = h->ph[r][i];
            if (p.used && hipEventElapsedTime(&t, p.e0, p.e1) == hipSuccess) { sum += t; ++used; }
        }
        ms[i] = used ? sum / used : -1.0;
    }
    return cnt;
}
GRAPE_BARRIER(h ? &h->err : &g_create_error)

int grape_reset_timings(grape_handle *h) try {
    if (!h) return GRAPE_ERR_INVALID;
    if (h->open) { h->open->ms_fwd = h->open->ms_bwd = 0.0; h->open->n_fwd = h->open->n_bwd = 0; return GRAPE_OK; }
    if (!h->shards.empty()) {
        for (grape_handle *c : h->shards) {
            const int rc = grape_reset_timings(c);
            if (rc) return multi_fail(h, c, rc);
        }
        h->host_enqueue_ms = 0.0;
        h->allreduce_ms = 0.0; h->allreduce_calls = 0;
        h->host_enqueue_calls = 0;
        return GRAPE_OK;
    }
    HIPCHK(h, hipSetDevice(h->device));
    HIPCHK(h, hipDeviceSynchronize());
    for (auto &ring : h->ph)
        for (auto &p : ring) p.used = false;
    h->n_fwd = h->n_bwd = 0;
    h->n_eval = 0;
    return GRAPE_OK;
}
GRAPE_BARRIER(h ? &h->err : &g_create_error)

int grape_get_work(grape_handle *h, double *out, int n) try {
    if (!h || !out || n < 4) return GRAPE_ERR_INVALID;
    if (h->open) return open_work(h, out, n);
    if (!h->shards.empty()) {
        const int m = n < 22 ? n : 22;
        std::fill(out, out + m, 0.0);
        for (grape_handle *c : h->shards) {
            double cw[22] = {0.};
            const int rc = grape_get_work(c, cw, m);
            if (rc < 0) return multi_fail(h, c, rc);
            for (int i = 0; i < m; ++i) out[i] = (i == 15 || i == 16 || i == 18) ? cw[i] : out[i] + cw[i];
        }
        if (m > 14 && out[14] > 0.0) out[14] = h->shards[0]->asm16p ? 3.0 : h->shards[0]->asm18gp ? 4.0 : h->shards[0]->asm18g ? 2.0 : 1.0;
        return 4;
    }
    HIPCHK(h, hipSetDevice(h->device));
    if (h->foreign_stream) HIPCHK(h, hipDeviceSynchronize());
    if (h->credit_pending) {
        ExpmArgs ea{};
        ea.H0f = h->d_H0f; ea.Hcf = h->d_Hcf; ea.eps = h->d_eps; ea.shape = h->d_shape; ea.dts = h->d_dts;
        ea.flags = h->d_flags; ea.stats = h->d_stats; ea.Sf = h->d_Sf;
        ea.K = h->KC; ea.rep = h->d_rep; ea.L = h->L; ea.N_T = h->N_T; ea.hc_per_traj = h->p.hc_per_traj;
        ea.n1 = h->d_n1; ea.n1_k = h->K;
        HIPCHK(h, (hipError_t)grape_t16_credit_launch(&ea, sizeof(ea), (void *)h->stream));
        HIPCHK(h, hipStreamSynchronize(h->stream));
        h->credit_pending = false;
    }
    unsigned long long sh[GRAPE_STAT_SHARDS * GRAPE_STAT_SLOTS], st[GRAPE_STAT_SLOTS] = {0};
    { const int rc_ = getter_fetch(h, sh, h->d_stats, sizeof(sh)); if (rc_) return rc_; }
    for (int q = 0; q < GRAPE_STAT_SHARDS; ++q)
        for (int i = 0; i < GRAPE_STAT_SLOTS; ++i) st[i] += sh[q * GRAPE_STAT_SLOTS + i];
    const double N3 = (double)h->N * h->N * h->N, N2 = (double)h->N * h->N;
    const double cells = (double)h->K * h->N_T, ecells = (double)h->KC * h->N_T;
    const double gemms = 2.0 * st[3] + 3.0 * st[4] + 4.0 * st[5] + 5.0 * st[6] + 6.0 * st[7];
    out[0] = cells;
    out[1] = (double)st[0];
    out[2] = (gemms + (double)st[0]) * 8.0 * N3 + ecells * (32.0 / 3.0) * N3;
    out[3] = (double)st[8] * (1.0 + 2.0 * h->L) * 8.0 * N2;
    if (n > 4) out[4] = (double)st[8];
    if (n > 5) out[5] = (double)st[9];
    if (n > 6) out[6] = h->series ? 0.0 : ecells;
    if (n > 7) out[7] = (double)st[10];
    if (n > 8) out[8] = (double)st[11];
    if (n > 9) out[9] = (double)st[12] * 2048.0;
    if (n > 10) out[10] = (double)st[13];
    if (n > 11) out[11] = (double)st[14];
    if (n > 12) out[12] = h->u_fallback ? 1.0 : 0.0;
    if (n > 13) out[13] = (double)st[15];
    if (n > 14) out[14] = h->asm16p ? 3.0 : h->asm16 ? 1.0 : h->asm18gp ? 4.0 : h->asm18g ? 2.0 : 0.0;
    if (n > 15) {
        double kind = 0.0;
        if (!h->series && h->d_park3 && h->NT == 4) {
            if (h->deriv3_general) kind = 3.0;
            else if (h->L > 2) kind = 2.0;
            else if (!h->deriv3_h0g && h->deriv3_asm) kind = 1.0;
        } else if (!h->series && h->deriv4_blocks) kind = 4.0;
        out[15] = kind;
    }
    if (n > 16) out[16] = (h->large && !h->series && h->t18 && h->lg_asm) ? 1.0 : 0.0;
    if (n > 17) {
        double carried = 0.0;
        if (h->last_walk_fuse && h->d_prog) {
            std::vector<int> prog((size_t)2 * h->K);
            { const int rc_ = getter_fetch(h, prog.data(), h->d_prog, prog.size() * sizeof(int)); if (rc_) return rc_; }
            for (int k = 0; k < h->K; ++k) {
                if (h->last_walk_fuse & 1) carried += prog[(size_t)k];
                if (h->last_walk_fuse & 2) carried += prog[(size_t)h->K + k];
            }
        }
        out[17] = carried;
    }
    if (n > 18) out[18] = h->scan16 ? (double)h->scan_Bk : 0.0;
    if (n > 19) {
        double certified = 0.0, seg = 0.0, qcells = 0.0;
        const bool want_seg = n > 20 && h->d_segplan && h->deriv_econ;
        const bool want_q = n > 21 && (h->asm16q || h->t16q_twin);
        if ((h->d_cert || want_seg || want_q) && h->d_splan && !h->series) {
            const size_t ncell = (size_t)h->KC * h->N_T;
            std::vector<int> plan(ncell);
            int fl[8];
            { const int rc_ = getter_fetch(h, plan.data(), h->d_splan, ncell * sizeof(int)); if (rc_) return rc_; }
            { const int rc_ = getter_fetch(h, fl, h->d_flags, sizeof(fl)); if (rc_) return rc_; }
            const bool tried = !(4L * fl[6] > (long)ncell);
            if (tried && h->d_cert)
                for (int w : plan) certified += (w & T16_PLAN_CERT) ? 1.0 : 0.0;
            if (tried && want_q)
                for (int w : plan) qcells += (w & T16_PLAN_Q) ? 1.0 : 0.0;
            if (tried && want_seg) {
                std::vector<int> sp(ncell), verdict(ncell);
                { const int rc_ = getter_fetch(h, sp.data(), h->d_segplan, ncell * sizeof(int)); if (rc_) return rc_; }
                { const int rc_ = getter_fetch(h, verdict.data(), h->d_cellflag, ncell * sizeof(int)); if (rc_) return rc_; }
                for (int k = 0; k < h->K; ++k) {
                    const size_t c0 = (size_t)(h->cls.empty() ? k : h->cls[k]) * h->N_T;
                    for (int i = 0; i < h->N_T; ++i)
                        seg += (sp[c0 + i] && verdict[c0 + i] == 0 && (plan[c0 + i] & T16_PLAN_SQ_MASK) == 0) ? 1.0 : 0.0;
                }
            }
        }
        out[19] = certified;
        if (n > 20) out[20] = seg;
        if (n > 21) out[21] = qcells;
    }
    return 4;
}
GRAPE_BARRIER(h ? &h->err : &g_create_error)

int grape_get_cert_table(grape_handle *h, int *dims, double *coef, int *exps) try {
    if (!h || !dims) return GRAPE_ERR_INVALID;
    if (h->open || !h->shards.empty()) {
        h->err = "grape_get_cert_table: a closed handle on one device";
        return GRAPE_ERR_INVALID;
    }
    const int nt = h->cert_n8 + h->cert_n6;
    dims[0] = h->KC; dims[1] = h->cert_n8; dims[2] = h->cert_n6;
    if (!h->d_cert || !nt) { dims[1] = dims[2] = 0; return GRAPE_OK; }
    HIPCHK(h, hipSetDevice(h->device));
    if (coef) HIPCHK(h, hipMemcpy(coef, h->d_cert, (size_t)h->KC * nt * sizeof(double), hipMemcpyDeviceToHost));
    if (exps) HIPCHK(h, hipMemcpy(exps, h->d_cert_exp, (size_t)nt * sizeof(int), hipMemcpyDeviceToHost));
    return GRAPE_OK;
}
GRAPE_BARRIER(h ? &h->err : &g_create_error)

int grape_get_seg_table(grape_handle *h, int *dims, double *coef, int *exps) try {
    if (!h || !dims) return GRAPE_ERR_INVALID;
    if (h->open || !h->shards.empty()) {
        h->err = "grape_get_seg_table: a closed handle on one device";
        return GRAPE_ERR_INVALID;
    }
    const int n4 = h->seg_n4, n8 = h->seg_n8, n12 = h->seg_n12, nt = n4 + n8 + n12;
    dims[0] = h->KC; dims[1] = n4; dims[2] = n8; dims[3] = n12;
    if (!h->d_seg || !nt) { dims[1] = dims[2] = dims[3] = 0; return GRAPE_OK; }
    HIPCHK(h, hipSetDevice(h->device));
    if (coef) {
        HIPCHK(h, hipMemcpy2D(coef, (size_t)nt * sizeof(double), h->d_seg, (size_t)(n4 + n12) * sizeof(double), (size_t)n4 * sizeof(double),
                              (size_t)h->KC, hipMemcpyDeviceToHost));
        HIPCHK(h, hipMemcpy2D(coef + n4, (size_t)nt * sizeof(double), h->d_seg8, (size_t)h->seg8_stride * sizeof(double), (size_t)n8 * sizeof(double),
                              (size_t)h->KC, hipMemcpyDeviceToHost));
        HIPCHK(h, hipMemcpy2D(coef + n4 + n8, (size_t)nt * sizeof(double), h->d_seg + n4, (size_t)(n4 + n12) * sizeof(double), (size_t)n12 * sizeof(double),
                              (size_t)h->KC, hipMemcpyDeviceToHost));
    }
    if (exps) {
        HIPCHK(h, hipMemcpy(exps, h->d_seg_exp + h->seg_exp_off, (size_t)n4 * sizeof(int), hipMemcpyDeviceToHost));
        HIPCHK(h, hipMemcpy(exps + n4, h->d_seg_exp, (size_t)n8 * sizeof(int), hipMemcpyDeviceToHost));
        HIPCHK(h, hipMemcpy(exps + n4 + n8, h->d_seg_exp + h->seg_exp_off + n4, (size_t)n12 * sizeof(int), hipMemcpyDeviceToHost));
    }
    return GRAPE_OK;
}
GRAPE_BARRIER(h ? &h->err : &g_create_error)

int grape_get_time_gradient(grape_handle *h, double *dJdt) try {
    if (h && h->open) return open_refuse(h, "grape_get_time_gradient");
    if (!h || !dJdt) return GRAPE_ERR_INVALID;
    const int N_T = h->N_T;
    if (!h->shards.empty()) {
        std::vector<double> part((size_t)N_T);
        for (size_t g = 0; g < h->shards.size(); ++g) {
            const int rc = grape_get_time_gradient(h->shards[g], g == 0 ? dJdt : part.data());
            if (rc) return multi_fail(h, h->shards[g], rc);
            if (g > 0) for (int n = 0; n < N_T; ++n) dJdt[n] += part[n];
        }
        return GRAPE_OK;
    }
    if (h->tg_state != 3) {
        h->err = h->tg_state == 0 ? "grape_get_time_gradient: no complete gradient evaluation on this time grid (none yet, the last "
                                    "one failed, or grape_set_tlist came after it)"
               : h->tg_state == 1 ? "grape_get_time_gradient: the last evaluation had no gradient (grape_eval with G == NULL)"
                                  : "grape_get_time_gradient called between grape_forward and the backward half";
        return GRAPE_ERR_INVALID;
    }
    HIPCHK(h, hipSetDevice(h->device));
    if (h->foreign_stream) HIPCHK(h, hipDeviceSynchronize());
    (void)hipGetLastError();
    if (!h->d_tq) HIPCHK(h, h->mem.alloc(&h->d_tq, (size_t)h->K * N_T));
    if (!h->d_dJdt) HIPCHK(h, h->mem.alloc(&h->d_dJdt, (size_t)N_T));
    TimeGradArgs ta{};
    ta.H0f = h->d_H0f; ta.Hcf = h->d_Hcf; ta.eps = h->d_eps; ta.shape = h->d_shape;
    ta.fw = h->d_fw; ta.bw = h->d_bw; ta.rho = h->d_rho; ta.z = h->tg_unit ? h->d_z : nullptr;
    ta.gb = (h->have_gb && !h->tg_xi_user) ? h->d_gb : nullptr; ta.lambda_q = 0.25 * h->p.lambda_b;
    ta.out = h->d_tq;
    ta.K = h->K; ta.L = h->L; ta.N = h->N; ta.NP = h->NP; ta.N_T = N_T; ta.hc_per_traj = h->p.hc_per_traj;
    const int nct = h->NP <= 64 ? 4 : h->NP <= 128 ? 2 : 1;
    const size_t lds = (size_t)2 * h->NP * 16 * nct * sizeof(double);
    const dim3 grid((unsigned)((N_T + 16 * nct - 1) / (16 * nct)), (unsigned)h->K);
    int dev = 0;
// ... 956 lines not shown
```

### grape.jl_amd/csrc/grape_t18.hip

```cpp
#include <hip/hip_runtime.h>
#include <stdint.h>
#include <string.h>
#include <type_traits>
#include <mutex>
#include <vector>
#include <stdlib.h>
#include <stdio.h>
namespace {
#include "grape_t18.hip.h"
#define GRAPE_BATCH_T18_UNIT
#include "grape_batch.hip.h"
#include "grape_deriv3.hip.h"
#include "grape_econ_coeffs.h"

template <int NT, bool SYM, bool CHEB, bool T16 = false>
hipError_t launch(const ExpmArgs &a, hipStream_t s, int blocks) {
    static size_t lds_set[64] = {0};
    const size_t lds = sizeof(double) * (size_t)T18Lds<NT>::TOTAL;
    int dev = 0;
    hipGetDevice(&dev);
    if (lds_set[dev & 63] < lds) {
        hipError_t e = hipFuncSetAttribute((const void *)expm_t18_kernel<NT, SYM, CHEB, T16>, hipFuncAttributeMaxDynamicSharedMemorySize, (int)lds);
        if (e != hipSuccess) return e;
        lds_set[dev & 63] = lds;
// ... 24 lines not shown
                                   int skip_if_flagged, int h0_general, int asm_ok, void *stream, int blocks) {
    if (d2size != sizeof(Deriv2Args)) return (int)hipErrorInvalidValue;
    Deriv3Args a;
    memcpy(&a.d, d2args, sizeof(a.d));
    a.H0f = H0f; a.Hcf = Hcf; a.wpt = wpt; a.skip_if_flagged = skip_if_flagged;
    hipStream_t s = (hipStream_t)stream;
    const int L = a.d.L;
    if (L < 1 || L > 8) return (int)hipErrorInvalidValue;
    if (h0_general == 2) {
        if (NT != 4 || skip_if_flagged || a.d.gpark) return (int)hipErrorInvalidValue;
        return (int)launch_d3_asm(a, s, blocks, true);
    }
    if (h0_general) {
        if (L > 2) return (int)hipErrorInvalidValue;
        if (NT == 3) return (int)(L == 1 ? launch_d3<3, 1, true>(a, s, blocks) : launch_d3<3, 2, true>(a, s, blocks));
        if (NT == 4) return (int)(L == 1 ? launch_d3<4, 1, true>(a, s, blocks) : launch_d3<4, 2, true>(a, s, blocks));
        return (int)hipErrorInvalidValue;
    }
#define D3_CASES(NT_)                                                                                                   \
    if (NT == NT_) {                                                                                                    \
        if (L == 1) return (int)launch_d3<NT_, 1>(a, s, blocks);                                                        \
        if (L == 2) return (int)launch_d3<NT_, 2>(a, s, blocks);                                                        \
        if (L <= 4) return (int)launch_d3<NT_, 4>(a, s, blocks);                                                        \
        return (int)launch_d3<NT_, 8>(a, s, blocks);                                                                    \
    }
    D3_CASES(1) D3_CASES(2) D3_CASES(3)
#undef D3_CASES
    if (NT == 4 && L > 2) {
        if (skip_if_flagged || a.d.gpark) return (int)hipErrorInvalidValue;
        return (int)launch_d3_asm(a, s, blocks);
    }
    if (NT == 4 && L <= 2) {
        if (asm_ok && !skip_if_flagged && !a.d.gpark) return (int)launch_d3_asm(a, s, blocks);
        return (int)(L == 1 ? launch_d3<4, 1>(a, s, blocks) : launch_d3<4, 2>(a, s, blocks));
    }
    return (int)hipErrorInvalidValue;
}

extern "C" const unsigned char grape_asm_co_start[], grape_asm_co_end[];
namespace {
struct T16AsmArgs {
    const double *H0f, *Sf, *dts;
    double2 *U;
    int *verdict;
    const int *rep;
    int KC, N_T, nblk;
    int fuse;
    unsigned long long *diag;
    const int *flags;
    const int *wgtab;
    const double2 *xinit;
    double2 *fw, *bw;
    int *prog;
    int K, s_per_cell;
    const int *splan;
};
static_assert(sizeof(T16AsmArgs) == 136, "argument block of the assembly kernel");

__device__ __forceinline__ double t16_post_norm1(const ExpmArgs &a, const int cell, double *red, const int tid) {
    constexpr int NP = 64;
    const int kc = cell / a.N_T, n = cell - kc * a.N_T, k = a.rep ? a.rep[kc] : kc;
    const double *h0 = a.H0f + (size_t)k * 2 * NP * NP, *sn = a.Sf + (size_t)(a.hc_per_traj ? cell : n) * 2 * NP * NP;
    const double dt = a.dts[n];
    const int j = tid & 63, part = tid >> 6;
    double sum = 0.;
    for (int i = part; i < NP; i += 4) {
        const double xr = dt * (h0[NP * NP + i * NP + j] + sn[NP * NP + i * NP + j]), xi = -dt * (h0[i * NP + j] + sn[i * NP + j]);
        sum += fast_sqrt(xr * xr + xi * xi);
    }
    red[tid] = sum;
    __syncthreads();
    if (tid < 64) {
        double c = red[tid] + red[64 + tid] + red[128 + tid] + red[192 + tid];
#pragma unroll
        for (int off = 32; off >= 1; off >>= 1) c = fmax(c, __shfl_xor(c, off, 64));
        if (tid == 0) red[256] = c;
    }
    __syncthreads();
    const double nA = red[256];
    __syncthreads();
    return nA;
}

__global__ void __launch_bounds__(256) t16_post_kernel(ExpmArgs a, const int *verdict, const int *prog, int nprog, const int *splan) {
    const int tid = threadIdx.x, lane = tid & 63, ncell = a.K * a.N_T;
    if (t16_skipped(a.flags, ncell)) return;
    if (prog && blockIdx.x == 0) {
        unsigned long long steps = 0;
        for (int i = tid; i < nprog; i += 256) steps += (unsigned long long)prog[i];
        for (int off = 32; off >= 1; off >>= 1) steps += __shfl_xor(steps, off, 64);
        if (lane == 0 && steps) stat_add(a.stats, 12, steps * 4ull * 2ull);
    }
    const int cell = blockIdx.x * 256 + tid;
    const bool valid = cell < ncell;
    const bool ok = valid && verdict[cell] == 0;
    if (valid && !ok) a.cell_list[atomicAdd(&a.flags[4], 1)] = cell;
    const unsigned long long m_ok = __ballot(ok), m_valid = __ballot(valid);
    {
        unsigned long long sq = valid ? (unsigned long long)(splan[cell] & T16_PLAN_SQ_MASK) : 0ull;
        unsigned long long sq_ok = ok ? sq : 0ull;
        for (int off = 32; off >= 1; off >>= 1) { sq += __shfl_xor(sq, off, 64); sq_ok += __shfl_xor(sq_ok, off, 64); }
        if (lane == 0 && sq) stat_add(a.stats, 12, sq * 4ull * 192ull);
        if (lane == 0 && sq_ok) stat_add(a.stats, 13, sq_ok);
    }
    const unsigned long long m_q = __ballot(valid && (splan[cell] & T16_PLAN_Q));
    if (lane == 0 && m_valid) {
        stat_add(a.stats, 12, (unsigned long long)__popcll(m_valid) * 4ull * (unsigned long long)(T16Count<4>::CELL + 1)
                                  - (unsigned long long)__popcll(m_q) * 4ull * (unsigned long long)(T18Count<4>::GP - T18Count<4>::SQH));
        if (m_ok) {
            stat_add(a.stats, 14, (unsigned long long)__popcll(m_ok));
            stat_add(a.stats, 15, (unsigned long long)__popcll(m_ok));
        }
        atomicAdd(&a.flags[5], (int)__popcll(m_valid));
    }
}

__global__ void __launch_bounds__(256) t16_credit_kernel(ExpmArgs a) {
    __shared__ double red[264];
    __shared__ int todo[256], ntodo;
    __shared__ unsigned long long cnt[8];
    const int tid = threadIdx.x, lane = tid & 63, ncell = a.K * a.N_T;
    if (t16_skipped(a.flags, ncell)) return;
    if (tid < 8) cnt[tid] = 0;
    if (tid == 0) ntodo = 0;
    __syncthreads();
    auto order_of = [](double nA) { return nA > 2.1 ? 4 : nA > 0.95 ? 3 : nA > 0.25 ? 2 : nA > 0.015 ? 1 : 0; };
    auto squarings_of = [](double nA) {
        if (!(nA > 5.4)) return 0;
        const double r = nA / 5.4;
        const int e = ilogb(r);
        return (r == ldexp(1.0, e)) ? e : e + 1;
    };
    const int cell = blockIdx.x * 256 + tid;
    bool cert = false;
    if (cell < ncell) {
        const double bound = expm_norm_bound(a, cell);
        cert = bound > 2.1 && bound <= 5.4;
        if (!cert) todo[atomicAdd(&ntodo, 1)] = cell;
    }
    const unsigned long long m_cert = __ballot(cert);
    if (lane == 0 && m_cert) atomicAdd(&cnt[2 + 4], (unsigned long long)__popcll(m_cert));
    __syncthreads();
    const int nt = ntodo;
    for (int q = 0; q < nt; ++q) {
        const double nA = t16_post_norm1(a, todo[q], red, tid);
        if (tid == 0) {
            const int sj = squarings_of(nA);
            if (sj) { cnt[0] += (unsigned long long)sj; cnt[1] = max(cnt[1], (unsigned long long)sj); }
            cnt[2 + order_of(nA)] += 1ull;
        }
    }
    __syncthreads();
    if (tid == 0) {
        if (cnt[0]) stat_add(a.stats, 0, cnt[0]);
        for (int o = 0; o < 5; ++o)
            if (cnt[2 + o]) stat_add(a.stats, 3 + o, cnt[2 + o]);
        if (cnt[1]) atomicMax(&a.flags[1], (int)cnt[1]);
    }
}

constexpr int D3_INV_TABLE = 2048;
constexpr int D3_PAIRS_OFF = 32768, D3_ECON_OFF = 32768, D3_ECON_TAB_B = 512;
struct AsmModule {
    hipModule_t mod = nullptr;
    hipFunction_t fn = nullptr, fn_d3 = nullptr, fn_d3s = nullptr, fn_lg = nullptr, fn_d3g = nullptr, fn_d4[2] = {nullptr, nullptr};
    hipFunction_t fn_t18g = nullptr, fn_t16p = nullptr, fn_t16p4 = nullptr, fn_t18gp = nullptr, fn_t16q = nullptr;
    double *inv = nullptr;
};
hipError_t asm_function(int dev, hipFunction_t *fn, hipFunction_t *fn_d3 = nullptr, const double **inv = nullptr,
                        hipFunction_t *fn_d3s = nullptr, hipFunction_t *fn_lg = nullptr, hipFunction_t *fn_d3g = nullptr,
                        hipFunction_t *fn_d4 = nullptr, int d4_index = 0, hipFunction_t *fn_t18g = nullptr,
                        hipFunction_t *fn_t16p = nullptr, int t16p_slots = 2, hipFunction_t *fn_t16q = nullptr) {
    static AsmModule mods[64];
    static std::mutex mtx;
    std::lock_guard<std::mutex> lock(mtx);
    AsmModule &m = mods[dev & 63];
    if (!m.fn) {
        static std::vector<char> override_co;
        const void *image = (const void *)grape_asm_co_start;
        if (const char *path = getenv("GRAPE_ASM_CO")) {
            if (override_co.empty()) {
                if (FILE *f = fopen(path, "rb")) {
                    fseek(f, 0, SEEK_END);
                    const long n = ftell(f);
                    fseek(f, 0, SEEK_SET);
                    if (n > 0) {
                        override_co.resize((size_t)n);
                        if (fread(override_co.data(), 1, (size_t)n, f) != (size_t)n) override_co.clear();
                    }
                    fclose(f);
                }
            }
            if (override_co.empty()) return hipErrorFileNotFound;
            image = override_co.data();
        }
        hipError_t e = hipModuleLoadData(&m.mod, image);
        if (e != hipSuccess) return e;
        e = hipModuleGetFunction(&m.fn_d3, m.mod, "deriv3_asm");
        if (e != hipSuccess) return e;
        e = hipModuleGetFunction(&m.fn_d3s, m.mod, "deriv3s_asm");
        if (e != hipSuccess) return e;
        e = hipModuleGetFunction(&m.fn_lg, m.mod, "lg_gemm_asm");
        if (e != hipSuccess) return e;
        e = hipModuleGetFunction(&m.fn_d3g, m.mod, "deriv3g_asm");
        if (e != hipSuccess) return e;
        e = hipModuleGetFunction(&m.fn_d4[0], m.mod, "deriv4_asm_128");
        if (e != hipSuccess) return e;
        e = hipModuleGetFunction(&m.fn_d4[1], m.mod, "deriv4_asm_256");
        if (e != hipSuccess) return e;
        e = hipModuleGetFunction(&m.fn_t18g, m.mod, "expm_t18g_asm");
        if (e != hipSuccess) return e;
        e = hipModuleGetFunction(&m.fn_t16p, m.mod, "expm_t16p_asm");
        if (e != hipSuccess) return e;
        e = hipModuleGetFunction(&m.fn_t16p4, m.mod, "expm_t16p4_asm");
        if (e != hipSuccess) return e;
        e = hipModuleGetFunction(&m.fn_t18gp, m.mod, "expm_t18gp_asm");
        if (e != hipSuccess) return e;
        e = hipModuleGetFunction(&m.fn_t16q, m.mod, "expm_t16q_asm");
        if (e != hipSuccess) return e;
        static_assert(D3_PAIRS_OFF >= (D3_INV_TABLE + 20) * 8 && D3_ECON_OFF == D3_INV_TABLE * 16 && ECON_MAXDEG - ECON_MINDEG <= 15, "layout of gen_d3.py");
        std::vector<double> tab((D3_PAIRS_OFF + D3_ECON_OFF + 16 * D3_ECON_TAB_B) / 8);
        tab[0] = 0.0;
        for (int i = 1; i < D3_INV_TABLE; ++i) tab[i] = 1.0 / (double)i;
        for (int a = 0; a < D3_INV_TABLE; ++a) tab[D3_PAIRS_OFF / 8 + 2 * a] = tab[D3_PAIRS_OFF / 8 + 2 * a + 1] = 1.0 / (double)(a + 1);
        for (int i = 0; i < ECON_NSETS; ++i)
            for (int a = 0; a < ECON_DEG[i]; ++a)
                for (int j = 0; j < 2; ++j)
                    tab[(D3_PAIRS_OFF + D3_ECON_OFF + (ECON_DEG[i] - ECON_MINDEG) * D3_ECON_TAB_B) / 8 + 2 * a + j] = ECON_TABS[i][a][j];
        int *pt = (int *)(tab.data() + D3_INV_TABLE);
        int np_ = 0;
        for (int ti = 0; ti < 4; ++ti)
            for (int tj = ti; tj < 4; ++tj)
                for (int plane = 0; plane < 2; ++plane)
                    for (int half = 0; half < 2; ++half) pt[np_++] = plane * 64 * 64 * 8 + ti * 16 * 64 * 8 + tj * 16 * 8;
        e = hipMalloc((void **)&m.inv, sizeof(double) * tab.size());
        if (e != hipSuccess) return e;
        e = hipMemcpy(m.inv, tab.data(), sizeof(double) * tab.size(), hipMemcpyHostToDevice);
        if (e != hipSuccess) return e;
        e = hipModuleGetFunction(&m.fn, m.mod, "expm_t16_asm");
        if (e != hipSuccess) return e;
    }
    if (fn) *fn = m.fn;
    if (fn_d3) *fn_d3 = m.fn_d3;
    if (fn_d3s) *fn_d3s = m.fn_d3s;
    if (fn_lg) *fn_lg = m.fn_lg;
    if (fn_d3g) *fn_d3g = m.fn_d3g;
    if (fn_d4) *fn_d4 = m.fn_d4[d4_index & 1];
    if (fn_t18g) *fn_t18g = m.fn_t18g;
    if (fn_t16p) *fn_t16p = t16p_slots == 4 ? m.fn_t16p4 : t16p_slots == 0 ? m.fn_t18gp : m.fn_t16p;
    if (fn_t16q) *fn_t16q = m.fn_t16q;
    if (inv) *inv = m.inv;
    return hipSuccess;
}
}

namespace {
struct D3AsmArgs {
    const double *H0f, *Hcf, *eps, *shape, *dts;
    const double2 *fw, *bw;
    const double *rho;
    double2 *tg;
    double *park;
    int *flags;
    unsigned long long *stats;
    const int *batch_flag;
    const double *inv;
    int K, L, N_T, hc_per_traj, wpt, batches_per_k, mcap, slots;
    double tol2;
    int deep, nblocks;
};
static_assert(sizeof(D3AsmArgs) == 160, "argument block of the assembly kernel");

hipError_t launch_d3_asm(const Deriv3Args &g, hipStream_t s, int blocks, bool general) {
    const Deriv2Args &a = g.d;
    if (a.L < 1 || a.L > (general ? 7 : 8) || blocks < 1 || a.maxm + 2 > D3_INV_TABLE) return hipErrorInvalidValue;
    if ((long)a.N_T + 1 >= (1L << 21) || (long)a.K * a.L * a.N_T >= (1L << 27)) return hipErrorInvalidValue;
    int dev = 0;
    hipError_t e = hipGetDevice(&dev);
    if (e != hipSuccess) return e;
    hipFunction_t fn, fn_s, fn_g;
    const double *inv;
    e = asm_function(dev, nullptr, &fn, &inv, &fn_s, nullptr, &fn_g);
    if (e != hipSuccess) return e;
    if (a.L > 2) fn = fn_s;
    if (general) fn = fn_g;
    D3AsmArgs k{};
    k.H0f = g.H0f; k.Hcf = g.Hcf; k.eps = a.eps; k.shape = a.shape; k.dts = a.dts; k.fw = a.fw; k.bw = a.bw; k.rho = a.rho;
    k.tg = a.tg; k.park = a.park; k.flags = a.flags; k.stats = a.stats; k.batch_flag = a.batch_flag; k.inv = inv;
    k.K = a.K; k.L = a.L; k.N_T = a.N_T; k.hc_per_traj = a.hc_per_traj; k.wpt = g.wpt; k.batches_per_k = a.batches_per_k;
    k.mcap = a.max_order < a.maxm ? a.max_order : a.maxm;
    k.slots = a.maxm + 1;
    k.tol2 = a.tol * a.tol;
    k.deep = (a.deep_redo && a.max_order > k.mcap) ? 1 : 0;
    if (a.batch_econ && !general && a.batch_flag && k.mcap >= ECON_MAXDEG) k.deep |= 2;
    k.nblocks = blocks;
    size_t size = sizeof(k);
    void *cfg[] = {HIP_LAUNCH_PARAM_BUFFER_POINTER, &k, HIP_LAUNCH_PARAM_BUFFER_SIZE, &size, HIP_LAUNCH_PARAM_END};
    return hipModuleLaunchKernel(fn, (unsigned)blocks, 1, 1, 256, 1, 1, 0, s, nullptr, cfg);
}
}

extern "C" const double *grape_econ_pairs(void) {
    int dev = 0;
    if (hipGetDevice(&dev) != hipSuccess) return nullptr;
    hipFunction_t fn;
    const double *inv = nullptr;
    if (asm_function(dev, nullptr, &fn, &inv) != hipSuccess || !inv) return nullptr;
    static_assert(D3_ECON_TAB_B == 64 * 8, "64 doubles per degree");
    return inv + (D3_PAIRS_OFF + D3_ECON_OFF) / 8;
}

namespace {
struct D4AsmArgs {
    const double *H0q, *Hcq, *H0p, *Hcp, *eps, *shape, *dts;
    const double2 *fw, *bw;
    const double *rho;
    double2 *tg;
    double *park;
    int *flags;
    unsigned long long *stats;
    const int *batch_flag;
    const double *inv;
    int K, L, N_T, hc_per_traj, nbatch_total, batches_per_k, mcap, slots;
    double tol2;
    int deep, nblocks;
};
static_assert(sizeof(D4AsmArgs) == 176, "argument block of the assembly kernel");
}
extern "C" int grape_deriv4_launch(int NP, const void *d2args, size_t d2size, const double *H0q3, const double *Hcq3, const double *H0p3,
                                   const double *Hcp3, void *stream, int blocks) {
    if (d2size != sizeof(Deriv2Args) || (NP != 128 && NP != 256) || blocks < 1) return (int)hipErrorInvalidValue;
    Deriv2Args a;
    memcpy(&a, d2args, sizeof(a));
    if (a.L < 1 || a.L > 8 || a.gpark || a.maxm + 2 > D3_INV_TABLE || !H0q3 || !Hcq3 || !H0p3 || !Hcp3) return (int)hipErrorInvalidValue;
    if ((long)a.N_T + 1 >= (1L << 19) || (long)a.K * a.L * a.N_T >= (1L << 27) || a.nbatch_total >= (1 << 24)) return (int)hipErrorInvalidValue;
    int dev = 0;
    hipError_t e = hipGetDevice(&dev);
    if (e != hipSuccess) return (int)e;
    hipFunction_t fn;
    const double *inv;
    e = asm_function(dev, nullptr, nullptr, &inv, nullptr, nullptr, nullptr, &fn, NP == 256);
    if (e != hipSuccess) return (int)e;
    D4AsmArgs k{};
    k.H0q = H0q3; k.Hcq = Hcq3; k.H0p = H0p3; k.Hcp = Hcp3; k.eps = a.eps; k.shape = a.shape; k.dts = a.dts; k.fw = a.fw; k.bw = a.bw;
    k.rho = a.rho; k.tg = a.tg; k.park = a.park; k.flags = a.flags; k.stats = a.stats; k.batch_flag = a.batch_flag; k.inv = inv;
    k.K = a.K; k.L = a.L; k.N_T = a.N_T; k.hc_per_traj = a.hc_per_traj; k.nbatch_total = a.nbatch_total; k.batches_per_k = a.batches_per_k;
    k.mcap = a.max_order < a.maxm ? a.max_order : a.maxm;
    k.slots = a.maxm + 1;
    k.tol2 = a.tol * a.tol;
    k.deep = (a.batch_econ && a.batch_flag && k.mcap >= ECON_MAXDEG) ? 2 : 0;
    k.nblocks = blocks;
    size_t size = sizeof(k);
    void *cfg[] = {HIP_LAUNCH_PARAM_BUFFER_POINTER, &k, HIP_LAUNCH_PARAM_BUFFER_SIZE, &size, HIP_LAUNCH_PARAM_END};
    return (int)hipModuleLaunchKernel(fn, (unsigned)blocks, 1, 1, 256, 1, 1, 0, (hipStream_t)stream, nullptr, cfg);
}

extern "C" int grape_lg_asm_launch(const void *k, size_t size, unsigned blocks, void *stream) {
    if (size != 416 || blocks == 0) return (int)hipErrorInvalidValue;
    int dev = 0;
    hipError_t e = hipGetDevice(&dev);
    if (e != hipSuccess) return (int)e;
    hipFunction_t fn;
    e = asm_function(dev, nullptr, nullptr, nullptr, nullptr, &fn);
    if (e != hipSuccess) return (int)e;
    unsigned char buf[416];
    memcpy(buf, k, sizeof(buf));
    size_t sz = sizeof(buf);
    void *cfg[] = {HIP_LAUNCH_PARAM_BUFFER_POINTER, buf, HIP_LAUNCH_PARAM_BUFFER_SIZE, &sz, HIP_LAUNCH_PARAM_END};
    return (int)hipModuleLaunchKernel(fn, blocks, 1, 1, 256, 1, 1, 0, (hipStream_t)stream, nullptr, cfg);
}

extern "C" void grape_t16_walks(int KC, int N_T, int nblk, int *tab) {
    const long ncell = (long)KC * N_T;
    for (int b = 0; b < nblk; ++b) {
        const long lo = b * ncell / nblk, hi = (b + 1) * ncell / nblk;
        int *e = tab + 4 * b;
        e[3] = 0;
        if (hi == lo) { e[0] = 0; e[1] = 0; e[2] = 1; }
        else if (lo % N_T == 0 || hi % N_T != 0) { e[0] = (int)lo; e[1] = (int)(hi - lo); e[2] = 1; }
        else { e[0] = (int)(hi - 1); e[1] = (int)(hi - lo); e[2] = -1; }
    }
}

extern "C" int grape_t16_asm_launch(const void *args, size_t args_size, int *verdict, void *stream, int blocks,
                                    const void *const *walk, int fuse, int K, int q) {
    if (args_size != sizeof(ExpmArgs)) return (int)hipErrorInvalidValue;
    ExpmArgs a;
    memcpy(&a, args, sizeof(a));
    if (!a.Sf || !verdict || blocks < 1 || !walk || !walk[0] || !walk[5]) return (int)hipErrorInvalidValue;
    if (fuse && (!walk[1] || !walk[2] || !walk[3] || !walk[4] || a.rep || K != a.K)) return (int)hipErrorInvalidValue;
    const long ncell = (long)a.K * a.N_T;
    if (ncell <= 0 || ncell >= (1L << 28)) return (int)hipErrorInvalidValue;
    int dev = 0;
    hipError_t e = hipGetDevice(&dev);
    if (e != hipSuccess) return (int)e;
    hipFunction_t fn, fn_q;
    e = asm_function(dev, &fn, nullptr, nullptr, nullptr, nullptr, nullptr, nullptr, 0, nullptr, nullptr, 2, &fn_q);
    if (e != hipSuccess) return (int)e;
    if (q) fn = fn_q;
    T16AsmArgs k{};
    k.H0f = a.H0f; k.Sf = a.Sf; k.dts = a.dts; k.U = a.U; k.verdict = verdict; k.rep = a.rep;
    k.KC = a.K; k.N_T = a.N_T; k.nblk = blocks; k.flags = a.flags;
    k.fuse = fuse; k.wgtab = (const int *)walk[0]; k.xinit = (const double2 *)walk[1]; k.fw = (double2 *)walk[2];
    k.bw = (double2 *)walk[3]; k.prog = (int *)walk[4]; k.K = K; k.splan = (const int *)walk[5];
    k.s_per_cell = a.hc_per_traj ? 1 : 0;
    size_t size = sizeof(k);
    void *cfg[] = {HIP_LAUNCH_PARAM_BUFFER_POINTER, &k, HIP_LAUNCH_PARAM_BUFFER_SIZE, &size, HIP_LAUNCH_PARAM_END};
    hipStream_t s = (hipStream_t)stream;
    e = hipModuleLaunchKernel(fn, (unsigned)blocks, 1, 1, 256, 1, 1, 0, s, nullptr, cfg);
    if (e != hipSuccess) return (int)e;
    hipLaunchKernelGGL(t16_post_kernel, dim3((unsigned)((ncell + 255) / 256)), dim3(256), 0, s, a, (const int *)verdict,
                       fuse ? (const int *)walk[4] : (const int *)nullptr, 2 * K, (const int *)walk[5]);
    return (int)hipGetLastError();
}

extern "C" int grape_t16p_asm_launch(const void *args, size_t args_size, int *verdict, void *stream, int blocks,
                                     const void *const *walk, int fuse, int K, const double *dte) {
    if (args_size != sizeof(ExpmArgs)) return (int)hipErrorInvalidValue;
    ExpmArgs a;
    memcpy(&a, args, sizeof(a));
    if (!a.hc_per_traj || a.L < 1 || a.L > 4 || !dte || !verdict || blocks < 1 || !walk || !walk[0] || !walk[5]) return (int)hipErrorInvalidValue;
    if (fuse && (!walk[1] || !walk[2] || !walk[3] || !walk[4] || a.rep || K != a.K)) return (int)hipErrorInvalidValue;
    const long ncell = (long)a.K * a.N_T;
    if (ncell <= 0 || ncell >= (1L << 28)) return (int)hipErrorInvalidValue;
    int dev = 0;
    hipError_t e = hipGetDevice(&dev);
    if (e != hipSuccess) return (int)e;
    hipFunction_t fn;
    e = asm_function(dev, nullptr, nullptr, nullptr, nullptr, nullptr, nullptr, nullptr, 0, nullptr, &fn, a.L <= 2 ? 2 : 4);
    if (e != hipSuccess) return (int)e;
    T16AsmArgs k{};
    k.H0f = a.H0f; k.Sf = a.Hcf; k.dts = dte; k.U = a.U; k.verdict = verdict; k.rep = a.rep;
    k.KC = a.K; k.N_T = a.N_T; k.nblk = blocks; k.flags = a.flags;
    k.fuse = fuse; k.wgtab = (const int *)walk[0]; k.xinit = (const double2 *)walk[1]; k.fw = (double2 *)walk[2];
    k.bw = (double2 *)walk[3]; k.prog = (int *)walk[4]; k.K = K; k.splan = (const int *)walk[5];
    k.s_per_cell = a.L;
    size_t size = sizeof(k);
    void *cfg[] = {HIP_LAUNCH_PARAM_BUFFER_POINTER, &k, HIP_LAUNCH_PARAM_BUFFER_SIZE, &size, HIP_LAUNCH_PARAM_END};
    hipStream_t s = (hipStream_t)stream;
    e = hipModuleLaunchKernel(fn, (unsigned)blocks, 1, 1, 256, 1, 1, 0, s, nullptr, cfg);
    if (e != hipSuccess) return (int)e;
    hipLaunchKernelGGL(t16_post_kernel, dim3((unsigned)((ncell + 255) / 256)), dim3(256), 0, s, a, (const int *)verdict,
                       fuse ? (const int *)walk[4] : (const int *)nullptr, 2 * K, (const int *)walk[5]);
    return (int)hipGetLastError();
}

namespace {
__global__ void __launch_bounds__(256) t18g_post_kernel(ExpmArgs a, const int *verdict, const int *prog, int nprog, const int *splan) {
    const int tid = threadIdx.x, lane = tid & 63, ncell = a.K * a.N_T;
    if (prog && blockIdx.x == 0) {
        unsigned long long steps = 0;
        for (int i = tid; i < nprog; i += 256) steps += (unsigned long long)prog[i];
        for (int off = 32; off >= 1; off >>= 1) steps += __shfl_xor(steps, off, 64);
        if (lane == 0 && steps) stat_add(a.stats, 12, steps * 4ull * 2ull);
    }
    const int cell = blockIdx.x * 256 + tid;
    const bool valid = cell < ncell;
    const bool bad = valid && verdict[cell] != 0;
    unsigned long long sq = valid ? (unsigned long long)splan[cell] : 0ull;
    for (int off = 32; off >= 1; off >>= 1) sq += __shfl_xor(sq, off, 64);
    const unsigned long long m_valid = __ballot(valid), m_bad = __ballot(bad);
    if (lane == 0 && m_valid) {
        const unsigned long long nc = (unsigned long long)__popcll(m_valid);
        stat_add(a.stats, 12, 4ull * (nc * (5ull * 192ull + 2ull) + sq * 192ull));
        if (sq) stat_add(a.stats, 13, sq);
        stat_add(a.stats, 14, nc);
        if (m_bad) atomicOr(&a.flags[0], 64);
    }
}
}

extern "C" int grape_t18g_asm_launch(const void *args, size_t args_size, int *verdict, void *stream, int blocks,
                                     const void *const *walk, int fuse, int K, const double *dte) {
    if (args_size != sizeof(ExpmArgs)) return (int)hipErrorInvalidValue;
    ExpmArgs a;
    memcpy(&a, args, sizeof(a));
    if ((!a.Sf && !dte) || !verdict || blocks < 1 || !walk || !walk[0] || !walk[5]) return (int)hipErrorInvalidValue;
    if (dte && (!a.hc_per_traj || a.L < 1 || a.L > 2)) return (int)hipErrorInvalidValue;
    if (fuse && (!walk[1] || !walk[2] || !walk[3] || !walk[4] || a.rep || K != a.K)) return (int)hipErrorInvalidValue;
    const long ncell = (long)a.K * a.N_T;
    if (ncell <= 0 || ncell >= (1L << 28)) return (int)hipErrorInvalidValue;
    int dev = 0;
    hipError_t e = hipGetDevice(&dev);
    if (e != hipSuccess) return (int)e;
    hipFunction_t fn;
    if (dte) e = asm_function(dev, nullptr, nullptr, nullptr, nullptr, nullptr, nullptr, nullptr, 0, nullptr, &fn, 0);
    else e = asm_function(dev, nullptr, nullptr, nullptr, nullptr, nullptr, nullptr, nullptr, 0, &fn);
    if (e != hipSuccess) return (int)e;
    T16AsmArgs k{};
    k.H0f = a.H0f; k.Sf = dte ? a.Hcf : a.Sf; k.dts = dte ? dte : a.dts; k.U = a.U; k.verdict = verdict; k.rep = a.rep;
    k.KC = a.K; k.N_T = a.N_T; k.nblk = blocks; k.flags = a.flags;
    k.fuse = fuse; k.wgtab = (const int *)walk[0]; k.xinit = (const double2 *)walk[1]; k.fw = (double2 *)walk[2];
    k.bw = (double2 *)walk[3]; k.prog = (int *)walk[4]; k.K = K; k.splan = (const int *)walk[5];
    k.s_per_cell = dte ? a.L : (a.hc_per_traj ? 1 : 0);
    size_t size = sizeof(k);
    void *cfg[] = {HIP_LAUNCH_PARAM_BUFFER_POINTER, &k, HIP_LAUNCH_PARAM_BUFFER_SIZE, &size, HIP_LAUNCH_PARAM_END};
    hipStream_t s = (hipStream_t)stream;
    e = hipModuleLaunchKernel(fn, (unsigned)blocks, 1, 1, 256, 1, 1, 0, s, nullptr, cfg);
    if (e != hipSuccess) return (int)e;
    hipLaunchKernelGGL(t18g_post_kernel, dim3((unsigned)((ncell + 255) / 256)), dim3(256), 0, s, a, (const int *)verdict,
                       fuse ? (const int *)walk[4] : (const int *)nullptr, 2 * K, (const int *)walk[5]);
    return (int)hipGetLastError();
}

extern "C" int grape_t16_credit_launch(const void *args, size_t args_size, void *stream) {
    if (args_size != sizeof(ExpmArgs)) return (int)hipErrorInvalidValue;
    ExpmArgs a;
    memcpy(&a, args, sizeof(a));
    if (!a.Sf) return (int)hipErrorInvalidValue;
    const long ncell = (long)a.K * a.N_T;
    hipLaunchKernelGGL(t16_credit_kernel, dim3((unsigned)((ncell + 255) / 256)), dim3(256), 0, (hipStream_t)stream, a);
    return (int)hipGetLastError();
}

extern "C" int grape_t18_launch(int NT, int herm, int t16, const void *args, size_t args_size, void *stream, int blocks) {
    if (args_size != sizeof(ExpmArgs)) return (int)hipErrorInvalidValue;
    ExpmArgs a;
    memcpy(&a, args, sizeof(a));
    hipStream_t s = (hipStream_t)stream;
    switch (NT) {
        case 1: return (int)(herm ? (t16 ? launch<1, false, true, true>(a, s, blocks) : launch<1, false, true>(a, s, blocks)) : launch<1, false, false>(a, s, blocks));
        case 2: return (int)(herm ? (t16 ? launch<2, false, true, true>(a, s, blocks) : launch<2, false, true>(a, s, blocks)) : launch<2, false, false>(a, s, blocks));
        case 3: return (int)(herm ? (t16 ? launch<3, true, true, true>(a, s, blocks) : launch<3, true, true>(a, s, blocks)) : launch<3, false, false>(a, s, blocks));
        default: return (int)(herm ? (t16 ? launch<4, true, true, true>(a, s, blocks) : launch<4, true, true>(a, s, blocks)) : launch<4, false, false>(a, s, blocks));
    }
}
// ... 28 lines not shown
```

Before: 58.96.

## Add t16r asm expm kernel overlapping A2 exchange and LDS reads with MFMAs

Adds a new generated gfx950 assembly kernel variant (t16r) derived from t16q. It moves the A2 add streams and LDS exchange writes into the tail of the first squaring product, and spreads the second product's LDS reads across MFMA gaps. It also drops the dummy bounding MFMA. The kernel is selected by default whenever t16q would be used, which removes serialised VALU and LDS phases between matrix products. The cost is a more complex instruction schedule, plus register allocation assumptions enforced only by asserts.

```diff
diff --git a/grape.jl_amd/api.py b/grape.jl_amd/api.py
--- a/grape.jl_amd/api.py
+++ b/grape.jl_amd/api.py
@@ -63,7 +63,7 @@
 def build_asm(verbose: bool = False, workdir: str | None = None) -> str:
     asm_dir = os.path.join(_CSRC, "asm")
     work = workdir or asm_dir
-    kernels = (("gen_t16.py", "expm_t16_asm"), ("gen_t16q.py", "expm_t16q_asm"), ("gen_t16p.py", "expm_t16p_asm"), ("gen_t16p.py", "expm_t16p4_asm"), ("gen_t18g.py", "expm_t18g_asm"), ("gen_t18gp.py", "expm_t18gp_asm"), ("gen_d3.py", "deriv3_asm"), ("gen_d3s.py", "deriv3s_asm"), ("gen_d3s.py", "deriv3g_asm"),
+    kernels = (("gen_t16.py", "expm_t16_asm"), ("gen_t16q.py", "expm_t16q_asm"), ("gen_t16r.py", "expm_t16r_asm"), ("gen_t16p.py", "expm_t16p_asm"), ("gen_t16p.py", "expm_t16p4_asm"), ("gen_t18g.py", "expm_t18g_asm"), ("gen_t18gp.py", "expm_t18gp_asm"), ("gen_d3.py", "deriv3_asm"), ("gen_d3s.py", "deriv3s_asm"), ("gen_d3s.py", "deriv3g_asm"),
                ("gen_lg.py", "lg_gemm_asm"), ("gen_d4.py", "deriv4_asm_128"), ("gen_d4.py", "deriv4_asm_256"))
     co_path, emb_s, emb_o = os.path.join(work, "grape_asm.co"), os.path.join(work, "asm_embed.S"), os.path.join(work, "asm_embed.o")
     llvm = "/opt/rocm/lib/llvm/bin"
@@ -95,7 +95,7 @@
 def _sources():
     srcs = [os.path.join(_CSRC, f) for f in ("grape_hip.hip", "grape_t18.hip", "grape_kernels.hip.h", "grape_large.hip.h",
                                              "grape_series.hip.h", "grape_cheby.hip.h", "grape_t18.hip.h", "grape_t18_coeffs.h",
-                                             "grape_deriv3.hip.h", "grape_timegrad.hip.h", "grape_batch.hip.h", "grape_lindblad.hip.h", "grape_lindblad_tg.hip.h", "grape_hvp.hip.h", "grape_hvp_split.hip.h", "grape_lindblad_hvp.hip.h", "grape_lindblad_hvp_split.hip.h", "grape_lindblad_batch.hip.h", "grape_lindblad_rc.hip.h", "grape_devmem.h", "grape_cert.hip.h", "grape_expect.hip.h", "grape_econ_coeffs.h", os.path.join("asm", "gen_t16.py"), os.path.join("asm", "gen_t16q.py"), os.path.join("asm", "gen_t16p.py"), os.path.join("asm", "gen_t18g.py"), os.path.join("asm", "gen_t18gp.py"), os.path.join("asm", "gen_d3.py"), os.path.join("asm", "gen_d3s.py"), os.path.join("asm", "gen_lg.py"), os.path.join("asm", "gen_d4.py"), os.path.join("asm", "gcn.py"))]
+                                             "grape_deriv3.hip.h", "grape_timegrad.hip.h", "grape_batch.hip.h", "grape_lindblad.hip.h", "grape_lindblad_tg.hip.h", "grape_hvp.hip.h", "grape_hvp_split.hip.h", "grape_lindblad_hvp.hip.h", "grape_lindblad_hvp_split.hip.h", "grape_lindblad_batch.hip.h", "grape_lindblad_rc.hip.h", "grape_devmem.h", "grape_cert.hip.h", "grape_expect.hip.h", "grape_econ_coeffs.h", os.path.join("asm", "gen_t16.py"), os.path.join("asm", "gen_t16q.py"), os.path.join("asm", "gen_t16r.py"), os.path.join("asm", "gen_t16p.py"), os.path.join("asm", "gen_t18g.py"), os.path.join("asm", "gen_t18gp.py"), os.path.join("asm", "gen_d3.py"), os.path.join("asm", "gen_d3s.py"), os.path.join("asm", "gen_lg.py"), os.path.join("asm", "gen_d4.py"), os.path.join("asm", "gcn.py"))]
     return srcs, os.path.join(_HERE, "..", "include", "grape_hip.h")
 
 
@@ -513,13 +513,14 @@
         self._chk(self._lib.grape_reset_timings(self._h))
 
     def work(self):
-        w = np.zeros(22)
-        self._lib.grape_get_work(self._h, w.ctypes.data, 22)
+        w = np.zeros(23)
+        self._lib.grape_get_work(self._h, w.ctypes.data, 23)
         return dict(cells=w[0], squarings=w[1], flop_expm=w[2], flop_deriv=w[3], deriv_orders=w[4],
                     pivoted_cells=w[5], expm_cells=w[6], series_terms=w[7], series_steps=w[8],
                     t18_mfma_flop=w[9], t18_squarings=w[10], t18_cells=w[11], matrix_free_fallback=w[12], t16_cells=w[13],
                     asm_kernel=w[14], asm_deriv_kernel=w[15], asm_blocked_products=w[16],
-                    walk_steps=w[17], scan_block=w[18], t16_certified=w[19], seg_certified=w[20], t16q_cells=w[21])
+                    walk_steps=w[17], scan_block=w[18], t16_certified=w[19], seg_certified=w[20], t16q_cells=w[21],
+                    t16r_kernel=w[22])
 
     def cert_table(self):
         dims = np.zeros(3, np.int32)
diff --git a/grape.jl_amd/csrc/asm/gen_t16.py b/grape.jl_amd/csrc/asm/gen_t16.py
--- a/grape.jl_amd/csrc/asm/gen_t16.py
+++ b/grape.jl_amd/csrc/asm/gen_t16.py
@@ -336,6 +336,7 @@
             p.valu("v_cndmask_b32", self.v_UO[r_], vidx, vpc, VCC)
         self.vp.free(t)
 
+    lead_ride = False
     early_free = False
 
     def pf_alloc(self):
@@ -479,7 +480,7 @@
         for t in (ta, tb, tc):
             self.vp.free(t)
 
-    def product(self, Q, B, half_last=False, init=None, hook=None, bload=None, fused=None):
+    def product(self, Q, B, half_last=False, init=None, hook=None, bload=None, fused=None, tail=None):
         p = self.p
         NS = len(Q)
         started = set(init or ())
@@ -526,6 +527,9 @@
                     for r in range(4 if so + 1 < NS else 0):
                         for pl in range(3):
                             gaps[max(last[pl], 3 * r + pl)].append(lambda pl=pl, r=r: rdk(pl, so + 1, r))
+                if so == 0 and fused.get("ride0"):
+                    for j, f in fused["ride0"]:
+                        gaps[j].append(f)
                 j = 0
                 for r in range(4):
                     for pl in range(3):
@@ -537,12 +541,24 @@
                 fused["post"]()
             p.s_barrier()
             sk0 = 1
+        pending = {}
         for pl in range(3):
-            for so in range(nslots(sk0)):
-                rd(pl, so, sk0, 0)
+            th = [lambda pl=pl, so=so: rd(pl, so, sk0, 0) for so in range(nslots(sk0))]
             if bload:
-                bload(pl, sk0, 0)
-        for sk in range(sk0, 4):
+                th.append(lambda pl=pl: bload(pl, sk0, 0))
+            if self.lead_ride and pl > 0:
+                pending[pl] = th
+            else:
+                for f in th:
+                    f()
+        if tail:
+            assert NS == 3 and half_last and sk0 < 3
+
+            def rdt(pl, so, r):
+                p.tag = "fragment"
+                p.ds_read(64, self.aop[pl][r], self.v_AA[so][3], self.KSTEP * r * LDB + pl * PLB)
+                p.tag = ""
+        for sk in range(sk0, 3 if tail else 4):
             for r in range(4):
                 ns = nslots(sk)
                 more = not (sk == 3 and r == 3)
@@ -553,10 +569,53 @@
                         mma(so, pl, self.aop[pl][so], B[pl][sk].d(r))
                         if hook and pl == 0 and so == 0:
                             hook(sk, r)
+                        if pending.get(pl + 1):
+                            pending[pl + 1].pop(0)()
+                    while pending.get(pl + 1):
+                        pending[pl + 1].pop(0)()
+                    if tail and nsk == 3:
+                        for r3 in range(4):
+                            rdt(pl, 1, r3)
+                            if bload:
+                                bload(pl, 3, r3)
+                        continue
                     for so in range(nsn):
                         rd(pl, so, nsk, nr)
                     if bload and more:
                         bload(pl, nsk, nr)
+        if tail:
+            for r in range(4):
+                for pl in range(3):
+                    mma(1, pl, self.aop[pl][r], B[pl][3].d(r))
+                    if hook and pl == 0:
+                        hook(3, r)
+                    rdt(pl, 0, r)
+            cut = tail.get("split_at", 12) if "split" in tail else 12
+
+            def spread(thunks, first, n):
+                gaps = [[] for _ in range(12)]
+                thunks = list(thunks or [])
+                if n <= 0:
+                    for f in thunks:
+                        f()
+                    return gaps
+                per = -(-len(thunks) // n)
+                for q, f in enumerate(thunks):
+                    gaps[first + q // per].append(f)
+                return gaps
+
+            gaps = spread(tail["mid"](), 0, cut)
+            j = 0
+            for r in range(4):
+                for pl in range(3):
+                    if j == cut and "split" in tail:
+                        gaps = spread(tail["split"](), cut, 12 - cut)
+                    mma(0, pl, self.aop[pl][r], B[pl][3].d(r))
+                    for f in gaps[j]:
+                        f()
+                    j += 1
+            if "split" in tail and cut == 12:
+                spread(tail["split"](), 12, 0)
 
     def plane_stores(self, sl, xr, xi, xs):
         if self.opts.get("nostore"):
@@ -620,6 +679,40 @@
     def load_c16(self, k16):
         self.smov64(k16, self.c["C16"])
 
+    def a2_streams(self, Qt, A2re, A2im, slots):
+        p = self.p
+        streams = []
+        for sl in slots:
+            for r in range(4):
+                p1, p2, p3 = (Qt[sl][j].d(r) for j in range(3))
+                re_, im_ = A2re[sl].d(r), A2im[sl].d(r)
+                streams.append([lambda re_=re_, p1=p1, p2=p2: p.valu("v_add_f64", re_, p1, Neg(p2)),
+                                lambda im_=im_, p3=p3, p1=p1: p.valu("v_add_f64", im_, p3, Neg(p1)),
+                                lambda im_=im_, p2=p2: p.valu("v_add_f64", im_, im_, Neg(p2))])
+        for g in range(0, len(streams), 4):
+            self.interleave(streams[g:g + 4])
+
+    def exchange_writes(self, re1, im1, re2, im2):
+        p = self.p
+        for r in range(4):
+            p.ds_write(64, self.v_EW2, re2.d(r), 128 * r)
+            p.ds_write(64, self.v_EW2, im2.d(r), EXH + 128 * r)
+            p.ds_write(64, self.v_EW1, re1.d(r), 128 * r)
+            p.ds_write(64, self.v_EW1, im1.d(r), EXH + 128 * r)
+
+    def first_square(self, Qt, B_As, hook_store, bload_A, Uprev):
+        p, vp, ap = self.p, self.vp, self.ap
+        self.product(Qt[:3], B_As, half_last=True, hook=hook_store, bload=bload_A)
+        ap.free(self.As_sm)
+        vp.free(Uprev)
+        self.stamp(1)
+        A2re, A2im, A2sm = [vp.alloc() for _ in range(4)], [vp.alloc() for _ in range(4)], [vp.alloc() for _ in range(4)]
+        self.a2_streams(Qt, A2re, A2im, range(3))
+        self.exchange_writes(A2re[1], A2im[1], A2re[2], A2im[2])
+        p.s_waitcnt(lgkm=0)
+        p.s_barrier()
+        return A2re, A2im, A2sm
+
     def cell(self):
         p, c = self.p, self.s_c
         vp, ap = self.vp, self.ap
@@ -648,10 +741,7 @@
                 p.tag = ""
 
         B_As = [[S_.sub(8 * sl, 8) for sl in range(4)] for S_ in As]
-        self.product(Qt[:3], B_As, half_last=True, hook=hook_store, bload=bload_A)
-        ap.free(self.As_sm)
-        vp.free(Uprev)
-        self.stamp(1)
+        A2re, A2im, A2sm = self.first_square(Qt, B_As, hook_store, bload_A, Uprev)
         As_re, As_im = self.As_re, self.As_im
 
         def A_(sl, r):
@@ -668,24 +758,6 @@
             for g in range(0, len(streams), 4):
                 self.interleave(streams[g:g + 4])
 
-        A2re, A2im, A2sm = [vp.alloc() for _ in range(4)], [vp.alloc() for _ in range(4)], [vp.alloc() for _ in range(4)]
-        streams = []
-        for sl in range(3):
-            for r in range(4):
-                p1, p2, p3 = (Qt[sl][j].d(r) for j in range(3))
-                re_, im_ = A2re[sl].d(r), A2im[sl].d(r)
-                streams.append([lambda re_=re_, p1=p1, p2=p2: p.valu("v_add_f64", re_, p1, Neg(p2)),
-                                lambda im_=im_, p3=p3, p1=p1: p.valu("v_add_f64", im_, p3, Neg(p1)),
-                                lambda im_=im_, p2=p2: p.valu("v_add_f64", im_, im_, Neg(p2))])
-        for g in range(0, len(streams), 4):
-            self.interleave(streams[g:g + 4])
-        for r in range(4):
-            p.ds_write(64, self.v_EW2, A2re[2].d(r), 128 * r)
-            p.ds_write(64, self.v_EW2, A2im[2].d(r), EXH + 128 * r)
-            p.ds_write(64, self.v_EW1, A2re[1].d(r), 128 * r)
-            p.ds_write(64, self.v_EW1, A2im[1].d(r), EXH + 128 * r)
-        p.s_waitcnt(lgkm=0)
-        p.s_barrier()
         cx = SimpleNamespace(Qt=Qt, A2re=A2re, A2im=A2im, A2sm=A2sm)
         self.second_product_fork(cx)
         self.advance()
diff --git a/grape.jl_amd/csrc/asm/gen_t16q.py b/grape.jl_amd/csrc/asm/gen_t16q.py
--- a/grape.jl_amd/csrc/asm/gen_t16q.py
+++ b/grape.jl_amd/csrc/asm/gen_t16q.py
@@ -49,6 +49,11 @@
         cx.pool = list(self.vp.free_tiles)
         p.salu("s_and_b32", self.s_tmp[0], self.s_scur, Q_BIT)
         p.s_branch("s_cbranch_scc1", cx.L_q)
+
+    def bound_stand_in(self, A2re):
+        drop = self.vp.alloc()
+        self.p.mfma(drop, A2re[0].d(0), A2re[0].d(0), 0)
+        self.vp.free(drop)
 
     def second_product_square(self, cx, L_join):
         p, vp = self.p, self.vp
@@ -114,9 +119,7 @@
             p.ds_read(128, txi.sub(4 * h, 4), self.v_ER, EXH + 16 * h)
             p.ds_read(128, Qt[3][0].sub(4 * h, 4), self.v_ER, (E2 - E1) + 16 * h)
             p.ds_read(128, Qt[3][2].sub(4 * h, 4), self.v_ER, (E2 - E1) + EXH + 16 * h)
-        drop = vp.alloc()
-        p.mfma(drop, A2re[0].d(0), A2re[0].d(0), 0)
-        vp.free(drop)
+        self.bound_stand_in(A2re)
         for r in range(4):
             p.valu("v_add_f64", Qt[2][0].d(r), Qt[2][0].d(r), txr.d(r))
             p.valu("v_add_f64", Qt[2][2].d(r), Qt[2][2].d(r), Neg(txi.d(r)))
diff --git a/grape.jl_amd/csrc/asm/gen_t16r.py b/grape.jl_amd/csrc/asm/gen_t16r.py
--- /dev/null
+++ b/grape.jl_amd/csrc/asm/gen_t16r.py
@@ -0,0 +1,171 @@
+import os
+import sys
+
+sys.path.insert(0, os.path.dirname(os.path.abspath(__file__)))
+from gcn import S, Neg, kernel_text
+from gen_t16 import E1, E2, EXH, LDS_BYTES, KERNARG
+from gen_t16q import GenQ
+
+HERE = os.path.dirname(os.path.abspath(__file__))
+MFMA_R = 120 + 120 + 2 * 192
+SPLIT2 = 6
+
+
+class GenR(GenQ):
+    def __init__(self, name="expm_t16r_asm", **kw):
+        super().__init__(name=name, **kw)
+        self.split2 = SPLIT2
+        self.lead_ride = not self.opts.get("nolead")
+        for o in self.opts:
+            if o.startswith("split2="):
+                self.split2 = int(o[7:])
+        assert 0 <= self.split2 <= 12
+
+    def bound_stand_in(self, A2re):
+        if self.opts.get("drop"):
+            super().bound_stand_in(A2re)
+
+    def exchange_thunks(self, re1, im1, re2, im2):
+        p = self.p
+        th = []
+        for r in range(4):
+            for addr, x, off in ((self.v_EW2, re2, 0), (self.v_EW2, im2, EXH), (self.v_EW1, re1, 0), (self.v_EW1, im1, EXH)):
+                th.append(lambda addr=addr, x=x, off=off, r=r: p.ds_write(64, addr, x.d(r), off + 128 * r))
+        return self.ride(th)
+
+    def ride(self, thunks):
+        if self.opts.get("bloc"):
+            for f in thunks:
+                f()
+            return []
+        return thunks
+
+    def first_square(self, Qt, B_As, hook_store, bload_A, Uprev):
+        if self.opts.get("x1late"):
+            return super().first_square(Qt, B_As, hook_store, bload_A, Uprev)
+        p, vp, ap = self.p, self.vp, self.ap
+        vp.free(Uprev)
+        A2re, A2im, A2sm = [vp.alloc() for _ in range(4)], [vp.alloc() for _ in range(4)], [vp.alloc() for _ in range(4)]
+        assert A2im[2].idx == Uprev.idx + 48 and A2sm[0].idx >= Uprev.idx + Uprev.n
+
+        def mid():
+            self.a2_streams(Qt, A2re, A2im, (2, 1))
+            return self.exchange_thunks(A2re[1], A2im[1], A2re[2], A2im[2])
+
+        self.product(Qt[:3], B_As, half_last=True, hook=hook_store, bload=bload_A, tail={"mid": mid})
+        ap.free(self.As_sm)
+        self.stamp(1)
+        self.a2_streams(Qt, A2re, A2im, (0,))
+        p.s_waitcnt(lgkm=0)
+        p.s_barrier()
+        return A2re, A2im, A2sm
+
+    def second_product_square(self, cx, L_join):
+        if self.opts.get("x2late"):
+            return super().second_product_square(cx, L_join)
+        p, vp = self.p, self.vp
+        Qt, A2re, A2im, A2sm = cx.Qt, cx.A2re, cx.A2im, cx.A2sm
+        p.s_branch("s_branch", L_join)
+        p.label(cx.L_q)
+        joined = list(vp.free_tiles)
+        vp.free_tiles[:] = cx.pool
+
+        self.advance()
+        self.cell_bases_issue(self.s_nkc, self.s_nn, self.s_ncell)
+        txr, txi = vp.alloc(), vp.alloc()
+        th = []
+        for h in range(2):
+            for dst, off in ((txr, 0), (txi, EXH), (A2re[3], E2 - E1), (A2im[3], (E2 - E1) + EXH)):
+                th.append(lambda dst=dst, off=off, h=h: p.ds_read(128, dst.sub(4 * h, 4), self.v_ER, off + 16 * h))
+        ride0 = []
+        if self.opts.get("noride0"):
+            for f in th:
+                f()
+        else:
+            ride0 = list(zip((0, 2, 3, 4, 6, 7, 8, 10), th))
+        self.stamp(2)
+        tx1 = (txr, txi)
+
+        def valu(sl):
+            if sl == 2:
+                for r in range(4):
+                    p.valu("v_add_f64", A2re[2].d(r), A2re[2].d(r), tx1[0].d(r))
+                    p.valu("v_add_f64", A2im[2].d(r), A2im[2].d(r), Neg(tx1[1].d(r)))
+                for r in range(4):
+                    p.valu("v_mul_f64", A2im[3].d(r), A2im[3].d(r), -1.0)
+                vp.free(tx1[0])
+                vp.free(tx1[1])
+            for r in range(4):
+                p.valu("v_add_f64", A2sm[sl].d(r), A2re[sl].d(r), A2im[sl].d(r))
+
+        kq = S(58, 2)
+
+        def y0_in_place(slots):
+            self.smov64(kq, self.cq["C1"])
+            streams = []
+            for sl in slots:
+                for r in range(4):
+                    p1, p2, p3 = (Qt[sl][j].d(r) for j in range(3))
+                    streams.append([lambda p3=p3, p1=p1: p.valu("v_add_f64", p3, p3, Neg(p1)),
+                                    lambda p1=p1, p2=p2: p.valu("v_add_f64", p1, p1, Neg(p2)),
+                                    lambda p3=p3, p2=p2: p.valu("v_add_f64", p3, p3, Neg(p2)),
+                                    lambda p1=p1: p.valu("v_mul_f64", p1, kq, p1),
+                                    lambda p3=p3: p.valu("v_mul_f64", p3, kq, p3)])
+            for g in range(0, len(streams), 4):
+                self.interleave(streams[g:g + 4])
+
+        def mid():
+            y0_in_place((2, 1))
+            return self.exchange_thunks(Qt[1][0], Qt[1][2], Qt[2][0], Qt[2][2])
+
+        tx2 = []
+
+        def split():
+            p.s_waitcnt(lgkm=0)
+            p.s_barrier()
+            xr, xi = vp.alloc(), vp.alloc()
+            tx2[:] = [xr, xi]
+            th = []
+            for h in range(2):
+                for dst, off in ((xr, 0), (xi, EXH), (Qt[3][0], E2 - E1), (Qt[3][2], (E2 - E1) + EXH)):
+                    th.append(lambda dst=dst, off=off, h=h: p.ds_read(128, dst.sub(4 * h, 4), self.v_ER, off + 16 * h))
+            return self.ride(th)
+
+        self.product(Qt[:3], [A2re, A2im, A2sm], half_last=True,
+                     fused={"valu": valu, "stores": lambda sl: self.plane_stores(sl, A2re[sl], A2im[sl], A2sm[sl]),
+                            "post": self.cell_coeffs(True), "ride0": ride0},
+                     tail={"mid": mid, "split": split, "split_at": self.split2})
+        for t in A2sm:
+            vp.free(t)
+        self.bound_stand_in(A2re)
+        self.cell_bases_finish(self.s_nkc)
+        self.stamp(3)
+        txr, txi = tx2
+        for r in range(4):
+            p.valu("v_add_f64", Qt[2][0].d(r), Qt[2][0].d(r), txr.d(r))
+            p.valu("v_add_f64", Qt[2][2].d(r), Qt[2][2].d(r), Neg(txi.d(r)))
+        for r in range(4):
+            p.valu("v_mul_f64", Qt[3][2].d(r), Qt[3][2].d(r), -1.0)
+        vp.free(txr)
+        vp.free(txi)
+        y0_in_place((0,))
+        p.salu("s_and_b32", self.s_prop, self.s_prop, 1)
+        self.stamp(4)
+        assert sorted(vp.free_tiles) == sorted(joined), (vp.free_tiles, joined)
+
+
+def generate(path=None, **kw):
+    g = GenR(**kw)
+    prog = g.build()
+    text = kernel_text(prog, KERNARG, LDS_BYTES)
+    if path:
+        with open(path, "w") as f:
+            f.write(text)
+    return g, prog, text
+
+
+if __name__ == "__main__":
+    out = sys.argv[1] if len(sys.argv) > 1 else os.path.join(HERE, "expm_t16r_asm.s")
+    g, prog, _ = generate(out)
+    print(f"{out}: {len(prog.ins)} lines, {prog.count('mfma')} matrix instructions, {prog.count('valu') + prog.count('dpp')} vector, "
+          f"{prog.count('lds')} LDS, {prog.count('vmem')} global, {prog.count('barrier')} barriers, {prog.auto_nops} wait states inserted")
diff --git a/grape.jl_amd/csrc/grape_hip.hip b/grape.jl_amd/csrc/grape_hip.hip
--- a/grape.jl_amd/csrc/grape_hip.hip
+++ b/grape.jl_amd/csrc/grape_hip.hip
@@ -122,6 +122,7 @@
     int *d_texp = nullptr;
     int t_n8 = 0, t_n6 = 0, t_n4 = 0, t_n12 = 0;
     bool asm16q = false;
+    bool asm16r = false;
     bool t16q_twin = false;
     bool asm16 = false;
     bool asm16p = false;
@@ -2848,6 +2849,8 @@
             const char *envt = getenv("GRAPE_EXPM_T16Q");
             const bool eligible = h->asm16 && !h->asm16p && !p->hc_per_traj && L >= 1 && L <= 2;
             h->asm16q = eligible && (envt ? atoi(envt) != 0 : ncell >= (long)T16Q_MIN_WALK * h->asm_blocks);
+            const char *envr = getenv("GRAPE_EXPM_T16R");
+            h->asm16r = h->asm16q && (envr ? atoi(envr) != 0 : !envt);
         }
         std::vector<int> tab((size_t)4 * h->asm_blocks);
         grape_t16_walks(h->KC, N_T, h->asm_blocks, tab.data());
@@ -3181,7 +3184,7 @@
                     walk_fuse = h->asm_walk & (1 | ((h->fuse && h->fuse_on && h->want_bw) ? 2 : 0));
                     if (walk_fuse) HIPCHK(h, stream_fill(h->d_prog, 0, (size_t)2 * h->K * sizeof(int), s));
                     const void *walk[6] = {h->d_wgtab, h->d_xinit, h->d_fw, h->d_bw, h->d_prog, h->d_splan};
-                    e = (hipError_t)grape_t16_asm_launch(&ea, sizeof(ea), h->d_cellflag, (void *)s, h->asm_blocks, walk, walk_fuse, h->K, h->asm16q ? 1 : 0);
+                    e = (hipError_t)grape_t16_asm_launch(&ea, sizeof(ea), h->d_cellflag, (void *)s, h->asm_blocks, walk, walk_fuse, h->K, h->asm16r ? 2 : h->asm16q ? 1 : 0);
                     h->credit_pending = true;
                 }
                 else {
@@ -4255,13 +4258,13 @@
     if (!h || !out || n < 4) return GRAPE_ERR_INVALID;
     if (h->open) return open_work(h, out, n);
     if (!h->shards.empty()) {
-        const int m = n < 22 ? n : 22;
+        const int m = n < 23 ? n : 23;
         std::fill(out, out + m, 0.0);
         for (grape_handle *c : h->shards) {
-            double cw[22] = {0.};
+            double cw[23] = {0.};
             const int rc = grape_get_work(c, cw, m);
             if (rc < 0) return multi_fail(h, c, rc);
-            for (int i = 0; i < m; ++i) out[i] = (i == 15 || i == 16 || i == 18) ? cw[i] : out[i] + cw[i];
+            for (int i = 0; i < m; ++i) out[i] = (i == 15 || i == 16 || i == 18 || i == 22) ? cw[i] : out[i] + cw[i];
         }
         if (m > 14 && out[14] > 0.0) out[14] = h->shards[0]->asm16p ? 3.0 : h->shards[0]->asm18gp ? 4.0 : h->shards[0]->asm18g ? 2.0 : 1.0;
         return 4;
@@ -4352,6 +4355,7 @@
         out[19] = certified;
         if (n > 20) out[20] = seg;
         if (n > 21) out[21] = qcells;
+        if (n > 22) out[22] = (h->asm16r && qcells > 0.0) ? 1.0 : 0.0;
     }
     return 4;
 }
diff --git a/grape.jl_amd/csrc/grape_t18.hip b/grape.jl_amd/csrc/grape_t18.hip
--- a/grape.jl_amd/csrc/grape_t18.hip
+++ b/grape.jl_amd/csrc/grape_t18.hip
@@ -130,7 +130,7 @@
     return nA;
 }
 
-__global__ void __launch_bounds__(256) t16_post_kernel(ExpmArgs a, const int *verdict, const int *prog, int nprog, const int *splan) {
+__global__ void __launch_bounds__(256) t16_post_kernel(ExpmArgs a, const int *verdict, const int *prog, int nprog, const int *splan, int q_stand_in) {
     const int tid = threadIdx.x, lane = tid & 63, ncell = a.K * a.N_T;
     if (t16_skipped(a.flags, ncell)) return;
     if (prog && blockIdx.x == 0) {
@@ -154,7 +154,7 @@
     const unsigned long long m_q = __ballot(valid && (splan[cell] & T16_PLAN_Q));
     if (lane == 0 && m_valid) {
         stat_add(a.stats, 12, (unsigned long long)__popcll(m_valid) * 4ull * (unsigned long long)(T16Count<4>::CELL + 1)
-                                  - (unsigned long long)__popcll(m_q) * 4ull * (unsigned long long)(T18Count<4>::GP - T18Count<4>::SQH));
+                                  - (unsigned long long)__popcll(m_q) * 4ull * (unsigned long long)(T18Count<4>::GP - T18Count<4>::SQH + (q_stand_in ? 0 : 1)));
         if (m_ok) {
             stat_add(a.stats, 14, (unsigned long long)__popcll(m_ok));
             stat_add(a.stats, 15, (unsigned long long)__popcll(m_ok));
@@ -212,13 +212,14 @@
 struct AsmModule {
     hipModule_t mod = nullptr;
     hipFunction_t fn = nullptr, fn_d3 = nullptr, fn_d3s = nullptr, fn_lg = nullptr, fn_d3g = nullptr, fn_d4[2] = {nullptr, nullptr};
-    hipFunction_t fn_t18g = nullptr, fn_t16p = nullptr, fn_t16p4 = nullptr, fn_t18gp = nullptr, fn_t16q = nullptr;
+    hipFunction_t fn_t18g = nullptr, fn_t16p = nullptr, fn_t16p4 = nullptr, fn_t18gp = nullptr, fn_t16q = nullptr, fn_t16r = nullptr;
     double *inv = nullptr;
 };
 hipError_t asm_function(int dev, hipFunction_t *fn, hipFunction_t *fn_d3 = nullptr, const double **inv = nullptr,
                         hipFunction_t *fn_d3s = nullptr, hipFunction_t *fn_lg = nullptr, hipFunction_t *fn_d3g = nullptr,
                         hipFunction_t *fn_d4 = nullptr, int d4_index = 0, hipFunction_t *fn_t18g = nullptr,
-                        hipFunction_t *fn_t16p = nullptr, int t16p_slots = 2, hipFunction_t *fn_t16q = nullptr) {
+                        hipFunction_t *fn_t16p = nullptr, int t16p_slots = 2, hipFunction_t *fn_t16q = nullptr,
+                        hipFunction_t *fn_t16r = nullptr) {
     static AsmModule mods[64];
     static std::mutex mtx;
     std::lock_guard<std::mutex> lock(mtx);
@@ -266,6 +267,8 @@
         if (e != hipSuccess) return e;
         e = hipModuleGetFunction(&m.fn_t16q, m.mod, "expm_t16q_asm");
         if (e != hipSuccess) return e;
+        e = hipModuleGetFunction(&m.fn_t16r, m.mod, "expm_t16r_asm");
+        if (e != hipSuccess) return e;
         static_assert(D3_PAIRS_OFF >= (D3_INV_TABLE + 20) * 8 && D3_ECON_OFF == D3_INV_TABLE * 16 && ECON_MAXDEG - ECON_MINDEG <= 15, "layout of gen_d3.py");
         std::vector<double> tab((D3_PAIRS_OFF + D3_ECON_OFF + 16 * D3_ECON_TAB_B) / 8);
         tab[0] = 0.0;
@@ -297,6 +300,7 @@
     if (fn_t18g) *fn_t18g = m.fn_t18g;
     if (fn_t16p) *fn_t16p = t16p_slots == 4 ? m.fn_t16p4 : t16p_slots == 0 ? m.fn_t18gp : m.fn_t16p;
     if (fn_t16q) *fn_t16q = m.fn_t16q;
+    if (fn_t16r) *fn_t16r = m.fn_t16r;
     if (inv) *inv = m.inv;
     return hipSuccess;
 }
@@ -442,10 +446,10 @@
     int dev = 0;
     hipError_t e = hipGetDevice(&dev);
     if (e != hipSuccess) return (int)e;
-    hipFunction_t fn, fn_q;
-    e = asm_function(dev, &fn, nullptr, nullptr, nullptr, nullptr, nullptr, nullptr, 0, nullptr, nullptr, 2, &fn_q);
-    if (e != hipSuccess) return (int)e;
-    if (q) fn = fn_q;
+    hipFunction_t fn, fn_q, fn_r;
+    e = asm_function(dev, &fn, nullptr, nullptr, nullptr, nullptr, nullptr, nullptr, 0, nullptr, nullptr, 2, &fn_q, &fn_r);
+    if (e != hipSuccess) return (int)e;
+    if (q) fn = q == 2 ? fn_r : fn_q;
     T16AsmArgs k{};
     k.H0f = a.H0f; k.Sf = a.Sf; k.dts = a.dts; k.U = a.U; k.verdict = verdict; k.rep = a.rep;
     k.KC = a.K; k.N_T = a.N_T; k.nblk = blocks; k.flags = a.flags;
@@ -458,7 +462,7 @@
     e = hipModuleLaunchKernel(fn, (unsigned)blocks, 1, 1, 256, 1, 1, 0, s, nullptr, cfg);
     if (e != hipSuccess) return (int)e;
     hipLaunchKernelGGL(t16_post_kernel, dim3((unsigned)((ncell + 255) / 256)), dim3(256), 0, s, a, (const int *)verdict,
-                       fuse ? (const int *)walk[4] : (const int *)nullptr, 2 * K, (const int *)walk[5]);
+                       fuse ? (const int *)walk[4] : (const int *)nullptr, 2 * K, (const int *)walk[5], q == 2 ? 0 : 1);
     return (int)hipGetLastError();
 }
 
@@ -489,7 +493,7 @@
     e = hipModuleLaunchKernel(fn, (unsigned)blocks, 1, 1, 256, 1, 1, 0, s, nullptr, cfg);
     if (e != hipSuccess) return (int)e;
     hipLaunchKernelGGL(t16_post_kernel, dim3((unsigned)((ncell + 255) / 256)), dim3(256), 0, s, a, (const int *)verdict,
-                       fuse ? (const int *)walk[4] : (const int *)nullptr, 2 * K, (const int *)walk[5]);
+                       fuse ? (const int *)walk[4] : (const int *)nullptr, 2 * K, (const int *)walk[5], 1);
     return (int)hipGetLastError();
 }
 
```

New measurement: 59.93, median of 6. 1.7% higher.
